# shubhamchandak94/Spring

Measured on AMD Instinct MI355X. Metric: Mreads/s through reorder stage, higher is better.
Workload: dtype u64; 1 GPU; 100000000 x 150 bp single-end synthetic reads per GPU (uniform genome 600000000 bp, 25x coverage, 1.0% substitutions, 50% reverse-complemented), inputs resident in HBM as .dna records; reads_per_gpu=100000000, read_len=150, chains=65536, num_thr=8, parallelism=single GPU, unmatched=13958636, singletons=12720853, rounds=1984, chain_groups=2

## Files before the change

include/spring_reorder.h:

```cpp
#ifndef SPRING_REORDER_H_
#define SPRING_REORDER_H_

#include <stddef.h>
#include <stdint.h>

#ifdef __cplusplus
extern "C" {
#endif

#define SPRING_REORDER_E_ARG (-1)
#define SPRING_REORDER_E_IO (-2)
#define SPRING_REORDER_E_HIP (-3)
#define SPRING_REORDER_E_STATE (-4)

typedef struct spring_reorder_ctx spring_reorder_ctx;

typedef struct {
  int32_t device;
  uint32_t num_chains;
  int32_t num_thr;
  int32_t collect_stats;
  int32_t time_search;
  int32_t force_literal_update;
  int32_t rounds_per_sync;
  int32_t long_budget;
  int32_t first_shifts;
  int32_t seed_wide;
  int32_t tab_scale;
  int32_t search_wpb;
  int32_t dbg_search_lds;
  int32_t dbg_apply_lds;
  int32_t fused;
  int32_t deep_bins;
  int32_t num_devices;
  int32_t devices[8];
  int32_t mg_host_transport;
  int32_t table_mode;
  int32_t plan0[6];
  int32_t plan1[6];
  int32_t long_min;
  int32_t long_blocks;
  int32_t debug;
  int32_t long_split;
  int32_t entry_flags;
  int32_t out_writers;
  int32_t alternatives;
  int32_t phases;
  int32_t known_absent;
} spring_reorder_opts;

typedef struct {
  uint64_t n_reads, n_matched, n_single, unmatched;
  uint64_t probes, keyok, cands, hits, iterations, rounds, lost;
  uint64_t numkeys[2], dict_numreads[2];
  double ms_unpack, ms_dict, ms_chains, ms_finalize, ms_total;
  double ms_search_kernel;
  uint64_t search_launches;
  uint64_t device_bytes;
  double ms_exchange, ms_resolve_mark;
  uint64_t chains;
  uint64_t deep_pool;
  uint64_t long_searches;
  uint64_t table_minz;
  uint64_t table_marked_lines;
  uint64_t long_splits;
  uint64_t alternatives;
  uint64_t phases;
  double ms_search_busy;
} spring_reorder_stats;

void spring_reorder_default_opts(spring_reorder_opts *o);
const char *spring_reorder_last_error(void);
void spring_reorder_trim_pool(void);

int spring_reorder_run(const char *temp_dir, uint32_t max_readlen, int32_t num_thr, int32_t paired_end,
                       uint32_t num_reads_clean_0, uint32_t num_reads_clean_1,
                       const spring_reorder_opts *opts );

int spring_reorder_create(spring_reorder_ctx **ctx, const spring_reorder_opts *opts);
void spring_reorder_destroy(spring_reorder_ctx *ctx);

int spring_reorder_load_dna(spring_reorder_ctx *ctx, const uint8_t *dna, size_t nbytes, uint32_t n,
                            uint32_t max_readlen);

int spring_reorder_load_dna_device(spring_reorder_ctx *ctx, const void *d_dna, size_t nbytes, uint32_t n,
                                   uint32_t max_readlen, int32_t fixed_len);

int spring_reorder_build_dict(spring_reorder_ctx *ctx);

int spring_reorder_run_chains(spring_reorder_ctx *ctx);
int spring_reorder_auto_chains(spring_reorder_ctx *ctx, uint32_t *chains, int32_t *deep);

typedef struct {
  uint32_t num_reads[2], num_reads_clean[2], num_reads_N[2];
  uint32_t max_readlen;
  uint32_t pad;
  double ms_device;
} spring_fastq_info;
int spring_reorder_load_fastq(spring_reorder_ctx *ctx, const uint8_t *fastq_1, size_t nbytes_1, const uint8_t *fastq_2,
                              size_t nbytes_2 , spring_fastq_info *info);
int spring_reorder_fastq_N(spring_reorder_ctx *ctx, int32_t which, uint8_t *n_dna, size_t cap, size_t *nbytes,
                           uint32_t *order_N, uint32_t *count);

int spring_reorder_mg_begin(spring_reorder_ctx *ctx, uint32_t rank, uint32_t world, uint32_t total_chains, void *d_prop);
int spring_reorder_mg_search(spring_reorder_ctx *ctx);
int spring_reorder_mg_slice(spring_reorder_ctx *ctx, void **d_prop, size_t *slice_off, size_t *slice_bytes,
                            size_t *total_bytes);
int spring_reorder_mg_slices(spring_reorder_ctx *ctx, void **d_prop, size_t slice_off[2], size_t slice_bytes[2],
                             size_t *total_bytes, uint32_t *count);
int spring_reorder_mg_apply(spring_reorder_ctx *ctx, int32_t check_alive, uint32_t *alive);
int spring_reorder_mg_end(spring_reorder_ctx *ctx);
int spring_reorder_debug_check_seed_state(spring_reorder_ctx *ctx, int32_t group, uint64_t *violations);
int spring_reorder_mg_exchange_virtual(spring_reorder_ctx **ctxs, uint32_t world);

#define SPRING_RCCL_ID_BYTES 128
typedef struct spring_mg_comm spring_mg_comm;
typedef int (*spring_mg_allgather_fn)(void *host_buf, size_t slice_off, size_t slice_bytes, size_t total_bytes,
                                      void *user);
int spring_mg_rccl_unique_id(void *id128);
int spring_mg_comm_create_rccl(spring_mg_comm **comm, int32_t device, const void *id128, uint32_t rank, uint32_t world);
int spring_mg_comm_create_host(spring_mg_comm **comm, spring_mg_allgather_fn fn, void *user, uint32_t rank,
                               uint32_t world);
void spring_mg_comm_destroy(spring_mg_comm *comm);
int spring_reorder_mg_run(spring_reorder_ctx *ctx, spring_mg_comm *comm, uint32_t total_chains);

int spring_reorder_finalize(spring_reorder_ctx *ctx);

int spring_reorder_get_stats(spring_reorder_ctx *ctx, spring_reorder_stats *st);

int spring_reorder_download(spring_reorder_ctx *ctx, uint32_t *order, char *rc, char *flag, int64_t *pos,
                            uint16_t *rlen, uint32_t *order_s, uint64_t *tid_off, uint64_t *tid_off_s);
int spring_reorder_tid_split(spring_reorder_ctx *ctx, uint64_t *mid, uint64_t *mid_s);

int spring_reorder_emit_dna(spring_reorder_ctx *ctx, int32_t tid, uint8_t *dst, size_t cap, size_t *nbytes);

int spring_reorder_dict_lookup(spring_reorder_ctx *ctx, int32_t which, const uint64_t *keys, uint32_t nkeys,
                               uint32_t *bin_size, uint32_t *bin_ids, size_t ids_cap);

int spring_reorder_download_reads(spring_reorder_ctx *ctx, uint64_t *limbs , uint16_t *len);

int spring_order_invert_se(const uint32_t *order, uint32_t n, uint32_t *order_array, double *kernel_ms);
int spring_order_invert_pe(const uint32_t *order, uint32_t n, uint32_t *order_array, double *kernel_ms);
int spring_order_correct(uint32_t *order, uint64_t m, const uint32_t *order_N, uint32_t nN, uint32_t n_clean,
                         double *kernel_ms);
int spring_order_pe_encode(const uint32_t *order, uint32_t n, uint32_t *new_order, double *kernel_ms);

int spring_fastq_reorder(const uint8_t *fastq, size_t nbytes, const uint32_t *order, uint32_t n, uint8_t *out,
                         size_t out_cap, size_t *out_bytes, double *kernel_ms);

#define SPRING_SYNTH_REPEATS 0x80000000u
#define SPRING_SYNTH_PAIRED 0x40000000u
#define SPRING_SYNTH_GENOMIC 0x20000000u
size_t spring_synth_dna_bytes(uint32_t n, uint32_t L);
int spring_synth_dna_host(uint8_t *dst, uint32_t n, uint32_t L, uint64_t G, uint64_t seed, uint32_t err_ppm);
int spring_synth_genome_host(uint8_t *dst, uint64_t G, uint64_t seed, uint32_t flags);
int spring_synth_dna_device(void *d_dst, uint32_t n, uint32_t L, uint64_t G, uint64_t seed, uint32_t err_ppm);
int spring_reorder_load_synth(spring_reorder_ctx *ctx, uint32_t n, uint32_t L, uint64_t G, uint64_t seed,
                              uint32_t err_ppm);
int spring_reorder_download_dna(spring_reorder_ctx *ctx, uint8_t *dst, size_t cap);

#ifdef __cplusplus
}
#endif
#endif
```

spring_amd/_lib.py:

```python
import ctypes as C
import os

HERE = os.path.dirname(os.path.abspath(__file__))
LIB_PATH = os.environ.get("SPRING_AMD_LIB") or os.path.join(HERE, "lib", "libspring_reorder_hip.so")

EXPORTS = [
    "spring_reorder_default_opts", "spring_reorder_last_error", "spring_reorder_trim_pool", "spring_reorder_run", "spring_reorder_create",
    "spring_reorder_destroy", "spring_reorder_load_dna", "spring_reorder_load_dna_device",
    "spring_reorder_build_dict", "spring_reorder_run_chains", "spring_reorder_auto_chains", "spring_reorder_finalize",
    "spring_reorder_mg_begin", "spring_reorder_mg_search", "spring_reorder_mg_slice", "spring_reorder_mg_slices",
    "spring_reorder_mg_apply",
    "spring_reorder_mg_end", "spring_reorder_mg_exchange_virtual", "spring_reorder_debug_check_seed_state",
    "spring_mg_rccl_unique_id", "spring_mg_comm_create_rccl", "spring_mg_comm_create_host", "spring_mg_comm_destroy",
    "spring_reorder_mg_run",
    "spring_reorder_get_stats", "spring_reorder_download", "spring_reorder_tid_split", "spring_reorder_emit_dna",
    "spring_reorder_dict_lookup", "spring_reorder_download_reads", "spring_synth_dna_bytes",
    "spring_reorder_load_fastq", "spring_reorder_fastq_N",
    "spring_order_invert_se", "spring_order_invert_pe", "spring_order_correct", "spring_order_pe_encode",
    "spring_fastq_reorder",
    "spring_synth_dna_host", "spring_synth_genome_host", "spring_synth_dna_device", "spring_reorder_load_synth", "spring_reorder_download_dna",
    "spring_encoder_create", "spring_encoder_destroy", "spring_encoder_set_split_tables", "spring_encoder_encode_reorder", "spring_encoder_download",
    "spring_encoder_download_seq_packed", "spring_encoder_get_info", "spring_reorder_encode_run", "spring_encoder_encode_host", "spring_encoder_run",
]

STREAMS_EXPORTS = [
    "spring_streams_create", "spring_streams_destroy", "spring_streams_from_encoder", "spring_streams_from_host",
    "spring_streams_download", "spring_streams_get_info", "spring_streams_run",
]
STREAMS_NUM = 9

DECODE_EXPORTS = [
    "spring_decode_create", "spring_decode_destroy", "spring_decode_seq_from_encoder", "spring_decode_seq_from_host",
    "spring_decode_seq_from_files", "spring_decode_from_streams", "spring_decode_from_host", "spring_decode_from_files",
    "spring_decode_download", "spring_decode_get_info",
]


class Opts(C.Structure):
    _fields_ = [("device", C.c_int32), ("num_chains", C.c_uint32), ("num_thr", C.c_int32),
                ("collect_stats", C.c_int32), ("time_search", C.c_int32), ("force_literal_update", C.c_int32),
                ("rounds_per_sync", C.c_int32), ("long_budget", C.c_int32),
                ("first_shifts", C.c_int32), ("seed_wide", C.c_int32), ("tab_scale", C.c_int32),
                ("search_wpb", C.c_int32), ("dbg_search_lds", C.c_int32), ("dbg_apply_lds", C.c_int32),
                ("fused", C.c_int32), ("deep_bins", C.c_int32),
                ("num_devices", C.c_int32), ("devices", C.c_int32 * 8), ("mg_host_transport", C.c_int32),
                ("table_mode", C.c_int32), ("plan0", C.c_int32 * 6), ("plan1", C.c_int32 * 6), ("long_min", C.c_int32),
                ("long_blocks", C.c_int32), ("debug", C.c_int32), ("long_split", C.c_int32), ("entry_flags", C.c_int32),
                ("out_writers", C.c_int32), ("alternatives", C.c_int32), ("phases", C.c_int32), ("known_absent", C.c_int32)]


class FastqInfo(C.Structure):
    _fields_ = [("num_reads", C.c_uint32 * 2), ("num_reads_clean", C.c_uint32 * 2), ("num_reads_N", C.c_uint32 * 2),
                ("max_readlen", C.c_uint32), ("pad", C.c_uint32), ("ms_device", C.c_double)]


class EncoderInfo(C.Structure):
    _fields_ = ([(k, C.c_uint64) for k in ("n_aligned", "n_total", "seq_len", "noise_bytes", "n_noisepos",
                                           "unaligned_bytes", "len_unaligned", "num_contigs")]
                + [(k, C.c_uint32) for k in ("matched_s", "matched_N", "align_passes", "max_bin")]
                + [("ms_device", C.c_double), ("ms_phase", C.c_double * 8)])

    def asdict(self):
        d = {}
        for k, _ in self._fields_:
            v = getattr(self, k)
            d[k] = list(v) if hasattr(v, "__len__") else v
        return d


class StreamsInfo(C.Structure):
    _fields_ = ([("num_units", C.c_uint64), ("num_blocks", C.c_uint64), ("bytes", C.c_uint64 * STREAMS_NUM),
                 ("flag_count", C.c_uint64 * 5), ("pos_escapes", C.c_uint64), ("n_aligned", C.c_uint64),
                 ("ms_device", C.c_double), ("ms_file", C.c_double)])

    def asdict(self):
        d = {}
        for k, _ in self._fields_:
            v = getattr(self, k)
            d[k] = list(v) if hasattr(v, "__len__") else v
        return d


class DecodeInfo(C.Structure):
    _fields_ = ([(k, C.c_uint64) for k in ("seq_len", "first_block", "num_blocks", "num_units")]
                + [("bases", C.c_uint64 * 2)]
                + [(k, C.c_uint64) for k in ("n_aligned", "n_unaligned", "pos_escapes")]
                + [("ms_device", C.c_double), ("ms_file", C.c_double)])

    def asdict(self):
        d = {}
        for k, _ in self._fields_:
            v = getattr(self, k)
            d[k] = list(v) if hasattr(v, "__len__") else v
        return d


class Stats(C.Structure):
    _fields_ = ([(k, C.c_uint64) for k in ("n_reads", "n_matched", "n_single", "unmatched", "probes", "keyok",
                                          "cands", "hits", "iterations", "rounds", "lost")]
                + [("numkeys", C.c_uint64 * 2), ("dict_numreads", C.c_uint64 * 2)]
                + [(k, C.c_double) for k in ("ms_unpack", "ms_dict", "ms_chains", "ms_finalize", "ms_total",
                                             "ms_search_kernel")]
                + [("search_launches", C.c_uint64), ("device_bytes", C.c_uint64),
                   ("ms_exchange", C.c_double), ("ms_resolve_mark", C.c_double), ("chains", C.c_uint64),
                   ("deep_pool", C.c_uint64), ("long_searches", C.c_uint64),
                   ("table_minz", C.c_uint64), ("table_marked_lines", C.c_uint64), ("long_splits", C.c_uint64), ("alternatives", C.c_uint64), ("phases", C.c_uint64),
                   ("ms_search_busy", C.c_double)])

    def asdict(self):
        d = {}
        for k, _ in self._fields_:
            v = getattr(self, k)
            d[k] = list(v) if hasattr(v, "__len__") else v
        return d


MG_ALLGATHER_FN = C.CFUNCTYPE(C.c_int, C.c_void_p, C.c_size_t, C.c_size_t, C.c_size_t, C.c_void_p)

_lib = None


def lib():
    global _lib
    if _lib is not None:
        return _lib
    if not os.path.exists(LIB_PATH):
        raise RuntimeError(
            "spring_amd: %s is missing. Build it with `python -m spring_amd.build` "
            "(or __graft_entry__.build()); there is no CPU fallback." % LIB_PATH)
    L = C.CDLL(LIB_PATH)
    vp, u8p = C.c_void_p, C.c_void_p
    L.spring_reorder_default_opts.argtypes = [C.POINTER(Opts)]
    L.spring_reorder_last_error.restype = C.c_char_p
    L.spring_reorder_trim_pool.restype = None
    L.spring_reorder_run.argtypes = [C.c_char_p, C.c_uint32, C.c_int32, C.c_int32, C.c_uint32, C.c_uint32,
                                     C.POINTER(Opts)]
    L.spring_reorder_create.argtypes = [C.POINTER(vp), C.POINTER(Opts)]
    L.spring_reorder_destroy.argtypes = [vp]
    L.spring_reorder_destroy.restype = None
    L.spring_reorder_load_dna.argtypes = [vp, u8p, C.c_size_t, C.c_uint32, C.c_uint32]
    L.spring_reorder_load_dna_device.argtypes = [vp, vp, C.c_size_t, C.c_uint32, C.c_uint32, C.c_int32]
    L.spring_reorder_build_dict.argtypes = [vp]
    L.spring_reorder_run_chains.argtypes = [vp]
    L.spring_reorder_auto_chains.argtypes = [vp, C.POINTER(C.c_uint32), C.POINTER(C.c_int32)]
    L.spring_reorder_finalize.argtypes = [vp]
    L.spring_reorder_mg_begin.argtypes = [vp, C.c_uint32, C.c_uint32, C.c_uint32, vp]
    L.spring_reorder_mg_search.argtypes = [vp]
    L.spring_reorder_mg_slice.argtypes = [vp, C.POINTER(vp), C.POINTER(C.c_size_t), C.POINTER(C.c_size_t), C.POINTER(C.c_size_t)]
    L.spring_reorder_mg_slices.argtypes = [vp, C.POINTER(vp), C.POINTER(C.c_size_t), C.POINTER(C.c_size_t), C.POINTER(C.c_size_t),
                                           C.POINTER(C.c_uint32)]
    L.spring_reorder_debug_check_seed_state.argtypes = [vp, C.c_int32, C.POINTER(C.c_uint64)]
    L.spring_reorder_mg_apply.argtypes = [vp, C.c_int32, C.POINTER(C.c_uint32)]
    L.spring_reorder_mg_end.argtypes = [vp]
    L.spring_reorder_mg_exchange_virtual.argtypes = [C.POINTER(vp), C.c_uint32]
    L.spring_mg_rccl_unique_id.argtypes = [vp]
    L.spring_mg_comm_create_rccl.argtypes = [C.POINTER(vp), C.c_int32, vp, C.c_uint32, C.c_uint32]
    L.spring_mg_comm_create_host.argtypes = [C.POINTER(vp), MG_ALLGATHER_FN, vp, C.c_uint32, C.c_uint32]
    L.spring_mg_comm_destroy.argtypes = [vp]
    L.spring_mg_comm_destroy.restype = None
    L.spring_reorder_mg_run.argtypes = [vp, vp, C.c_uint32]
    L.spring_reorder_get_stats.argtypes = [vp, C.POINTER(Stats)]
    L.spring_reorder_download.argtypes = [vp] + [vp] * 8
    L.spring_reorder_tid_split.argtypes = [vp, vp, vp]
    L.spring_reorder_emit_dna.argtypes = [vp, C.c_int32, u8p, C.c_size_t, C.POINTER(C.c_size_t)]
    L.spring_reorder_dict_lookup.argtypes = [vp, C.c_int32, vp, C.c_uint32, vp, vp, C.c_size_t]
    L.spring_reorder_download_reads.argtypes = [vp, vp, vp]
    L.spring_reorder_load_fastq.argtypes = [vp, vp, C.c_size_t, vp, C.c_size_t, C.POINTER(FastqInfo)]
    L.spring_reorder_fastq_N.argtypes = [vp, C.c_int32, vp, C.c_size_t, C.POINTER(C.c_size_t), vp, C.POINTER(C.c_uint32)]
    L.spring_order_invert_se.argtypes = [vp, C.c_uint32, vp, C.POINTER(C.c_double)]
    L.spring_order_invert_pe.argtypes = [vp, C.c_uint32, vp, C.POINTER(C.c_double)]
    L.spring_fastq_reorder.argtypes = [u8p, C.c_size_t, vp, C.c_uint32, u8p, C.c_size_t, C.POINTER(C.c_size_t),
                                       C.POINTER(C.c_double)]
    L.spring_order_pe_encode.argtypes = [vp, C.c_uint32, vp, C.POINTER(C.c_double)]
    L.spring_order_correct.argtypes = [vp, C.c_uint64, vp, C.c_uint32, C.c_uint32, C.POINTER(C.c_double)]
    L.spring_synth_dna_bytes.restype = C.c_size_t
    L.spring_synth_dna_bytes.argtypes = [C.c_uint32, C.c_uint32]
    L.spring_synth_dna_host.argtypes = [u8p, C.c_uint32, C.c_uint32, C.c_uint64, C.c_uint64, C.c_uint32]
    L.spring_synth_genome_host.argtypes = [u8p, C.c_uint64, C.c_uint64, C.c_uint32]
    L.spring_synth_dna_device.argtypes = [vp, C.c_uint32, C.c_uint32, C.c_uint64, C.c_uint64, C.c_uint32]
    L.spring_reorder_load_synth.argtypes = [vp, C.c_uint32, C.c_uint32, C.c_uint64, C.c_uint64, C.c_uint32]
    L.spring_reorder_download_dna.argtypes = [vp, u8p, C.c_size_t]
    L.spring_encoder_create.argtypes = [C.c_int32, C.POINTER(vp)]
    L.spring_encoder_destroy.argtypes = [vp]
    L.spring_encoder_destroy.restype = None
    L.spring_encoder_encode_reorder.argtypes = [vp, vp, u8p, C.c_uint64, vp, C.c_uint32, C.POINTER(EncoderInfo)]
    L.spring_encoder_download.argtypes = [vp] + [vp] * 9
    L.spring_encoder_download_seq_packed.argtypes = [vp, vp, vp]
    L.spring_encoder_encode_host.argtypes = [vp, C.c_uint32, C.c_int32, vp, u8p, C.c_uint64, vp, vp, vp, vp, vp, u8p,
                                             C.c_uint64, vp, C.c_uint32, u8p, C.c_uint64, vp, C.c_uint32,
                                             C.POINTER(EncoderInfo)]
    L.spring_encoder_run.argtypes = [C.c_char_p, C.c_uint32, C.c_int32, C.c_uint32, C.c_uint32, C.c_int32,
                                     C.POINTER(EncoderInfo)]
    L.spring_encoder_get_info.argtypes = [vp, C.POINTER(EncoderInfo)]
    L.spring_reorder_encode_run.argtypes = [C.c_char_p, C.c_uint32, C.c_int32, C.c_int32, C.c_uint32, C.c_uint32,
                                            C.c_uint32, C.POINTER(Opts), C.POINTER(EncoderInfo)]
    L.spring_streams_create.argtypes = [C.c_int32, C.POINTER(vp)]
    L.spring_streams_destroy.argtypes = [vp]
    L.spring_streams_destroy.restype = None
    L.spring_streams_from_encoder.argtypes = [vp, vp, C.c_uint32, C.c_int32, C.c_int32, C.c_uint32, C.c_int32,
                                              C.POINTER(StreamsInfo)]
    L.spring_streams_from_host.argtypes = [vp, vp, vp, C.c_uint64, vp, C.c_uint64, vp, C.c_uint64, vp, vp, C.c_uint64, vp,
                                           C.c_uint64, C.c_uint32, C.c_int32, C.c_int32, C.c_uint32, C.POINTER(StreamsInfo)]
    L.spring_streams_download.argtypes = [vp, C.c_int32, vp, vp]
    L.spring_streams_get_info.argtypes = [vp, C.POINTER(StreamsInfo)]
    L.spring_streams_run.argtypes = [C.c_char_p, C.c_uint32, C.c_int32, C.c_int32, C.c_uint32, C.c_int32,
                                     C.POINTER(StreamsInfo)]
    L.spring_decode_create.argtypes = [C.c_int32, C.POINTER(vp)]
    L.spring_decode_destroy.argtypes = [vp]
    L.spring_decode_destroy.restype = None
    L.spring_decode_seq_from_encoder.argtypes = [vp, vp]
    L.spring_decode_seq_from_host.argtypes = [vp, C.c_int32, vp, vp, vp]
    L.spring_decode_seq_from_files.argtypes = [vp, C.c_char_p, C.c_int32]
    L.spring_decode_from_streams.argtypes = [vp, vp, C.POINTER(DecodeInfo)]
    L.spring_decode_from_host.argtypes = [vp, vp, vp, C.c_uint32, C.c_uint32, C.c_uint32, C.c_int32, C.c_int32,
                                          C.c_uint32, C.POINTER(DecodeInfo)]
    L.spring_decode_from_files.argtypes = [vp, C.c_char_p, C.c_uint32, C.c_uint32, C.c_uint32, C.c_int32, C.c_int32,
                                           C.c_uint32, C.POINTER(DecodeInfo)]
    L.spring_decode_download.argtypes = [vp, C.c_int32, vp, vp]
    L.spring_decode_get_info.argtypes = [vp, C.POINTER(DecodeInfo)]
    for name in DECODE_EXPORTS:
        if name != "spring_decode_destroy":
            getattr(L, name).restype = C.c_int
    for name in STREAMS_EXPORTS:
        if name != "spring_streams_destroy":
            getattr(L, name).restype = C.c_int
    for name in EXPORTS:
        if name not in ("spring_reorder_last_error", "spring_reorder_destroy", "spring_synth_dna_bytes",
                        "spring_reorder_default_opts", "spring_reorder_trim_pool", "spring_encoder_destroy",
                        "spring_mg_comm_destroy"):
            getattr(L, name).restype = C.c_int
    _lib = L
    return L
```

spring_amd/csrc/reorder_device.h:

```cpp
#ifndef SPRING_REORDER_DEVICE_H_
#define SPRING_REORDER_DEVICE_H_

#include <hip/hip_runtime.h>
#include <stdint.h>

namespace sr {

constexpr int MAX_READ_LEN = 511;
constexpr int MAX_SEARCH = 1000;
constexpr int THRESH = 4;
constexpr uint32_t DEEP_BIN = 16;
constexpr uint32_t MID_BIN = 64;
constexpr uint32_t BIG_BIN = 256;
constexpr uint32_t CHUNK = 64;
constexpr uint32_t MARK_BLOCK = 256;
constexpr uint32_t MC_WAVES_PER_BLOCK = MARK_BLOCK / 4 + 3;
constexpr int UBLK_SHIFT = 12;
constexpr int LDS_PAD = 10;
constexpr int LDS_LIMBS = 16 + 2 * LDS_PAD;

enum { MODE_SEARCH = 0, MODE_NEED_SEED = 1 };
enum { PROP_NONE = 0, PROP_MATCH = 1, PROP_SEED = 2, PROP_FRESH = 3  };
enum { PK_NONE = 0, PK_MATCH = 1, PK_SEED = 2, PK_NOSEED = 4, PK_DONE = 5 };
constexpr unsigned long long PK_CURSOR_BIT = 1ull << 35;
constexpr unsigned long long PK_WILLNEED_BIT = 1ull << 36;
constexpr int PK_ALT_SHIFT = 37;
constexpr uint32_t ALT_MAX_READS = (1u << 27) - 1;
constexpr uint32_t ALT_KEY = 1u << 28;

struct __attribute__((aligned(16))) ChainHot {
  long long ref_pos;
  int32_t ref_len;
  uint32_t e_slot;
  uint32_t prev, first_rid;
  uint32_t n_emit, n_single;
  uint32_t s_slot;
  uint32_t num_reads_thr, num_unmatched_past;
  uint32_t prop_rid;
  union {
    struct {
      uint32_t done : 1, prev_unmatched : 1, left_search : 1, stop_searching : 1;
      uint32_t mode : 1, retrying : 1, finishing : 1, cursor_writer : 1;
      uint32_t cnt_buf : 1;
      uint32_t cnt_wide : 1;
      uint32_t prop_kind : 2;
      uint32_t prop_rev : 3;
      uint32_t prop_shift : 9;
    };
    uint32_t flags;
  };
  uint32_t alt1;
  uint32_t pad[2];
};
static_assert(sizeof(ChainHot) == 64, "ChainHot must be one 64-byte line");

struct __attribute__((aligned(64))) Chain {
  ChainHot h;
  uint64_t ref[16];
  uint64_t revref[16];
  uint64_t st_probes, st_keyok, st_cands, st_iter, st_lost, st_hits, n_unmatched, st_long ;
#ifdef SR_PHASE_TIMING
  uint64_t pt[64];
#endif
};
#ifndef SR_PHASE_TIMING
static_assert(sizeof(Chain) == 384, "Chain layout");
#endif

struct Globals {
  long long cursor;
  uint32_t alive;
  uint32_t e_alloc;
  uint32_t s_alloc;
  uint32_t pad;
  long long cursor_b;
};

struct TabView {
  const uint4 *buck;
  int bshift;
  int minz;
  int lshift;
};
constexpr uint32_t TAG_MARK = 0xfffffffcu;
constexpr int MINZ_HEAVY = 12;
constexpr int MINZ_K = 16;
constexpr int MINZ_WL = 32;

constexpr int LONG_MAX_BINS = 1024;
constexpr int LONG_MAX_PARTS = 64;
struct LongHead {
  uint32_t nb, nparts, best_single, bestrid;
  uint32_t bestpart, pad[3];
  uint32_t blo[LONG_MAX_PARTS + 4];
  uint32_t rescode[LONG_MAX_PARTS], resrid[LONG_MAX_PARTS];
  uint32_t capped[LONG_MAX_PARTS];
};
struct DevParams {
  const uint64_t *reads;
  const uint16_t *lens;
  uint32_t n;
  int L, W, S, Lpad, maxshift, uniform_len;
  int plan[2][6];
  int seed_wide;
  int deep_bins;
  int search_wpb;
  int dbg_search_lds, dbg_apply_lds;
  int wl;
  int dstart[2], dend[2];
  uint32_t numkeys[2];
  TabView tab;
  const ulonglong2 *urec[2];
  const uint32_t *ids[2];
  uint32_t *epos[2];
  uint32_t idmask;
  const ulonglong2 *sig[2];
  uint64_t *taken;
  uint32_t *ublk;
  uint32_t *resv;
  uint32_t *needy;
  uint32_t *needy_cnt;
  uint32_t *needy_cnt_next;
  int fused;
  int alts;
  int mc;
  int ka, ka_lo;
  uint32_t *ord;
  uint4 *ord_cnt;
  uint32_t *longq;
  int long_budget, long_min, long_blocks, long_part;
  uint32_t *lctl, *lparts;
  struct LongHead *lhead;
  uint2 *lbin;
  uint16_t *lbcode;
  uint32_t lbin_stride;
#ifdef SR_PHASE_TIMING
  unsigned long long *dbg;
#endif
  Globals *glob;
  long long *cursor;
  uint32_t K, c0, Ktot;
  int phases;
  uint32_t g0, Kg, g0_other, Kg_other;
  uint32_t gg0, gKg, gKg_other;
  uint32_t seed_lo, seed_hi;
  uint32_t nb_lo, nb_hi;
  const uint64_t *taken_other;
  uint32_t *won, *won_other;
  unsigned long long *prop;
  uint32_t *alive_wave;
  Chain *chains;
  int4 *cnt;
  uint32_t *cnt8;
  uint4 *e_rec; uint2 *e_chunk;
  uint32_t *s_rec; uint2 *s_chunk;
  uint32_t *f_order; char *f_rc; char *f_flag; long long *f_pos; uint16_t *f_len; uint32_t *f_order_s;
};

void launch_unpack(hipStream_t st, const uint8_t *dna, const uint64_t *off, uint32_t n, int L, int W, int S,
                   uint32_t rec_fixed, uint64_t *reads, uint16_t *lens, uint32_t *bad_len = nullptr);
void launch_flag_in_dict(hipStream_t st, const uint16_t *lens, uint32_t n, int dend, uint32_t *flag);
void launch_keys(hipStream_t st, const uint64_t *reads, const uint16_t *lens, const uint32_t *slot, uint32_t n,
                 int S, int dstart, int dend, uint64_t *keys, uint32_t *vals);
struct DictBuild {
  const uint32_t *ustart, *ucount, *ids;
  ulonglong2 *urec;
  uint32_t *deep, *ndeep;
};
void launch_tab_insert(hipStream_t st, const uint64_t *mhash, const uint64_t *mval, uint64_t nmerged, DictBuild d0,
                       DictBuild d1, uint32_t *fpt, int bshift);
void launch_minz_prepare(hipStream_t st, const uint64_t *mhash, const uint64_t *mval, uint64_t nmerged, DictBuild d0,
                         DictBuild d1, int lshift, uint32_t *bucket, uint64_t *tagpay);
void launch_tab_insert_minz(hipStream_t st, const uint32_t *bucket_sorted, const uint64_t *tagpay_sorted, uint64_t nmerged,
                            uint32_t *fpt, int bshift, uint32_t *marked);
hipError_t sort_pairs_u32_u64(hipStream_t st, void *tmp, size_t &tmp_bytes, const uint32_t *kin, uint32_t *kout,
                              const uint64_t *vin, uint64_t *vout, size_t n, unsigned end_bit);
hipError_t merge_by_hash(hipStream_t st, void *tmp, size_t &tmp_bytes, const uint64_t *k0, const uint64_t *k1,
                         const uint64_t *v0, const uint64_t *v1, uint64_t *kout, uint64_t *vout, size_t n0, size_t n1);
void launch_iota_tag(hipStream_t st, uint64_t *v, uint64_t n, uint64_t tag);
void launch_build_epos(hipStream_t st, const uint32_t *ids, uint64_t m, uint32_t *epos);
void launch_trim_bins(hipStream_t st, const uint32_t *deep, const uint32_t *ndeep, uint32_t ndeep_host,
                      ulonglong2 *urec, const uint32_t *ids, const uint64_t *taken, ulonglong2 *sig ,
                      uint32_t *epos = nullptr );
void launch_build_sig(hipStream_t st, const uint32_t *ids, uint64_t m, const uint64_t *reads, int S, int W, ulonglong2 *sig);
void launch_dict_lookup(hipStream_t st, TabView tab, const ulonglong2 *urec, int which,
                        const uint64_t *reads, int S, int dstart, int dend, const uint64_t *keys, uint32_t nkeys,
                        uint32_t *start, uint32_t *count);
void launch_fill_u32(hipStream_t st, uint32_t *p, uint64_t n, uint32_t v);
void launch_init_taken(hipStream_t st, uint64_t *taken, uint64_t nwords, uint32_t n, uint32_t *ublk);
void launch_init_chains(hipStream_t st, const DevParams &P, bool seeds = true);
void launch_check_seed_state(hipStream_t st, const DevParams &P, uint64_t nwords, uint64_t hi, unsigned long long *bad);
void launch_search(hipStream_t st, const DevParams &P, bool stats);
void launch_apply(hipStream_t st, const DevParams &P, bool literal);
void launch_round(hipStream_t st, const DevParams &P, bool stats, bool mg);
void launch_mg_resolve(hipStream_t st, const DevParams &P);
void launch_mg_mark(hipStream_t st, const DevParams &P);
void launch_ph_mark(hipStream_t st, const DevParams &P);
void launch_delay(hipStream_t st, uint32_t microseconds);
void launch_chain_summary(hipStream_t st, const DevParams &P, uint2 *sum, unsigned long long *tot );
void launch_scatter(hipStream_t st, const DevParams &P, uint64_t cap_m, uint64_t cap_s, const uint64_t *off_m,
                    const uint64_t *off_s);
void launch_rec_size(hipStream_t st, const uint32_t *order, const uint16_t *lens, uint64_t cnt, uint32_t *sz);
void launch_emit_dna(hipStream_t st, const uint64_t *reads, const uint16_t *lens, int S, const uint32_t *order,
                     const char *rc, uint64_t cnt, const uint64_t *off, uint32_t rec_fixed, uint8_t *dst);
void launch_synth(hipStream_t st, uint8_t *dst, uint32_t n, uint32_t L, uint64_t G, uint64_t seed, uint32_t thr24);

constexpr int NL_CHUNK_BYTES = 4096;
void launch_nl_count(hipStream_t st, const uint8_t *t, uint64_t nbytes, uint32_t *blk_cnt, uint64_t nblk);
void launch_nl_fill(hipStream_t st, const uint8_t *t, uint64_t nbytes, const uint64_t *blk_off, uint64_t *line_end,
                    uint64_t nblk);
void launch_read_info(hipStream_t st, const uint8_t *t, const uint64_t *line_end, uint64_t nreads, uint32_t *len,
                      uint32_t *fclean, uint32_t *szc, uint32_t *fN, uint32_t *szN, uint32_t *lenc, uint32_t *err);
void launch_pack_reads(hipStream_t st, const uint8_t *t, const uint64_t *line_end, uint64_t nreads, const uint32_t *len,
                       const uint32_t *fclean, const uint32_t *cidx, const uint64_t *coff, const uint32_t *nidx,
                       const uint64_t *noff, uint32_t cidx_base, uint64_t coff_base, uint32_t file_read_base,
                       uint8_t *out_clean, uint64_t *out_off, uint8_t *out_N, uint32_t *out_orderN, uint64_t *out_offN);
hipError_t reduce_max_u32(hipStream_t st, void *tmp, size_t &tmp_bytes, const uint32_t *in, uint32_t *out, size_t n);
hipError_t reduce_min_u32(hipStream_t st, void *tmp, size_t &tmp_bytes, const uint32_t *in, uint32_t *out, size_t n);

hipError_t sort_pairs(hipStream_t st, void *tmp, size_t &tmp_bytes, const uint64_t *kin, uint64_t *kout,
                      const uint32_t *vin, uint32_t *vout, size_t n, unsigned end_bit);
hipError_t rle(hipStream_t st, void *tmp, size_t &tmp_bytes, const uint64_t *in, size_t n, uint64_t *uniq,
               uint32_t *counts, uint32_t *nruns);
hipError_t excl_scan_u32(hipStream_t st, void *tmp, size_t &tmp_bytes, const uint32_t *in, uint32_t *out, size_t n);
hipError_t excl_scan_u32_to_u64(hipStream_t st, void *tmp, size_t &tmp_bytes, const uint32_t *in, uint64_t *out,
                                size_t n);

}
#endif
```

spring_amd/csrc/reorder_kernels.hip:

```cpp
#include <cstdlib>
#include <cstring>
#include <hip/hip_runtime.h>
#include <rocprim/rocprim.hpp>

#include "reorder_device.h"
#include "synth_common.h"

namespace sr {


__device__ __forceinline__ uint64_t mix64(uint64_t x) {
  x ^= x >> 33; x *= 0xff51afd7ed558ccdull; x ^= x >> 33; x *= 0xc4ceb9fe1a85ec53ull; x ^= x >> 33;
  return x;
}

__device__ __forceinline__ void wave_sync() {
  __builtin_amdgcn_fence(__ATOMIC_SEQ_CST, "wavefront");
  __builtin_amdgcn_wave_barrier();
}

__device__ __forceinline__ int uni_i32(int v) { return __builtin_amdgcn_readfirstlane(v); }
template <class T>
__device__ __forceinline__ T *uni_ptr(T *p) {
  const uint64_t a = reinterpret_cast<uint64_t>(p);
// ... 31 lines not shown
__device__ __forceinline__ uint64_t lds_window(const uint64_t *s, int bitpos) {
  int li = bitpos >> 6, off = bitpos & 63;
  uint64_t lo = s[li], hi = s[li + 1];
  return off ? (lo >> off) | (hi << (64 - off)) : lo;
}

__device__ __forceinline__ bool is_taken(const uint64_t *__restrict__ taken, uint32_t rid) {
  return (taken[rid >> 6] >> (rid & 63)) & 1ull;
}
__device__ __forceinline__ bool entry_dead(const DevParams &P, uint32_t &r, bool &trimmable) {
  if (P.idmask != 0xffffffffu) {
    const bool f = (r >> 31) != 0;
    r &= 0x7fffffffu;
    trimmable = f;
    if (f || P.phases != 2) return f;
    return is_taken(P.taken, r);
  }
  const bool d = is_taken(P.taken, r);
  trimmable = d && (P.phases != 2 || is_taken(P.taken_other, r));
  return d;
}

__device__ __forceinline__ uint32_t fp30_of(uint64_t h) {
  const uint32_t f = (uint32_t)h & 0x3fffffffu;
  return f == 0u ? 1u : f == 0x3fffffffu ? 0x3ffffffeu : f;
}
__device__ __forceinline__ uint64_t bucket_of(uint64_t h, int bshift) { return h >> bshift; }
__device__ __forceinline__ uint64_t bucket_mask(int bshift) { return (1ull << (64 - bshift)) - 1; }
__device__ __forceinline__ uint64_t unmix64(uint64_t x) {
  x ^= x >> 33; x *= 0x9cb4b2f8129337dbull; x ^= x >> 33; x *= 0x4f74430c22a54005ull; x ^= x >> 33;
  return x;
}
__device__ __forceinline__ uint32_t fmix32(uint32_t x) {
  x ^= x >> 16; x *= 0x85ebca6bu; x ^= x >> 13; x *= 0xc2b2ae35u; x ^= x >> 16;
  return x;
}
__device__ __forceinline__ uint32_t kmer_order(uint32_t x) {
  uint32_t r = __builtin_bitreverse32(x);
  r = ~(((r >> 1) & 0x55555555u) | ((r & 0x55555555u) << 1));
  return ((x < r ? x : r) ^ 0x5bd1e995u) * 0x9e3779b1u;
}
__device__ __forceinline__ uint32_t minz_of_key(uint64_t key) {
  uint32_t m = 0xffffffffu;
#pragma unroll
  for (int q = 0; q <= MINZ_WL - MINZ_K; q++) m = min(m, kmer_order((uint32_t)(key >> (2 * q))));
  return fmix32(m);
}
__device__ __forceinline__ uint64_t tab_home(const TabView &T, uint64_t h, uint32_t mz) {
  return T.minz ? (((uint64_t)(mz >> T.lshift) << 2) | ((h >> 30) & 3ull)) : bucket_of(h, T.bshift);
}
__device__ __forceinline__ uint64_t tab_redirect_x(uint32_t x32, int bshift) { return mix64(0x6a09e667f3bcc908ull ^ x32) >> bshift; }
__device__ __forceinline__ uint64_t tab_redirect(const TabView &T, uint64_t h) {
  return tab_redirect_x(fp30_of(h) | ((uint32_t)((h >> 30) & 3ull) << 30), T.bshift);
}
template <bool MZ = false>
__device__ __forceinline__ int tab_find(const TabView &T, uint64_t h, uint32_t mz, int l, int skip,
                                        uint32_t &pay, bool &other) {
  const uint32_t mine = (fp30_of(h) << 2) | ((uint32_t)l << 1), theirs = mine ^ 2u;
  const uint64_t bmask = bucket_mask(T.bshift);
  uint64_t b = MZ ? tab_home(T, h, mz) : bucket_of(h, T.bshift);
  bool first = MZ && T.minz != 0;
  for (;;) {
#if defined(SR_TAGS_NT)
    typedef uint32_t u32x4_t __attribute__((ext_vector_type(4)));
    const u32x4_t tv = __builtin_nontemporal_load(reinterpret_cast<const u32x4_t *>(&T.buck[b * 2]));
    const uint4 t = make_uint4(tv.x, tv.y, tv.z, tv.w);
#elif defined(SR_TAGS_SC)
    typedef uint32_t u32x4_t __attribute__((ext_vector_type(4)));
    u32x4_t tv;
    asm volatile("global_load_dwordx4 %0, %1, off sc0 sc1\n\ts_waitcnt vmcnt(0)" : "=v"(tv) : "v"(&T.buck[b * 2]) : "memory");
    const uint4 t = make_uint4(tv.x, tv.y, tv.z, tv.w);
#else
    const uint4 t = T.buck[b * 2];
#endif
    if (MZ && first) {
      first = false;
      if (t.x == TAG_MARK) { b = tab_redirect(T, h); continue; }
    }
    other = other || (t.x & ~1u) == theirs || (t.y & ~1u) == theirs || (t.z & ~1u) == theirs || t.w != 0;
    uint32_t m = (uint32_t)((t.x & ~1u) == mine) | ((uint32_t)((t.y & ~1u) == mine) << 1) |
                 ((uint32_t)((t.z & ~1u) == mine) << 2) | ((uint32_t)((t.w & ~1u) == mine) << 3);
    const int c = __popc(m);
    if (c > skip) {
      for (; skip > 0; skip--) m &= m - 1;
      const int I = __ffs((int)m) - 1;
      const uint32_t Tg = I == 0 ? t.x : I == 1 ? t.y : I == 2 ? t.z : t.w;
      pay = reinterpret_cast<const uint32_t *>(T.buck)[b * 8 + 4 + I];
      return 1 + (int)(Tg & 1u);
    }
    if (t.w == 0) return 0;
    skip -= c;
    b = (b + 1) & bmask;
  }
}
__device__ __forceinline__ uint64_t read_window(const uint64_t *__restrict__ r, int S, int dstart, int klen2) {
  const int bitpos = 2 * dstart, li = bitpos >> 6, off = bitpos & 63;
  uint64_t v = r[li] >> off;
  if (off && li + 1 < S) v |= r[li + 1] << (64 - off);
  if (klen2 < 64) v &= (1ull << klen2) - 1;
  return v;
}

#ifdef SR_PHASE_TIMING
#ifndef SR_PT_LONG
#define SR_PT_LONG 1000000
#endif
__shared__ uint32_t g_pt_lds[66];
#define PT(k)                                                                                         \
  do {                                                                                                \
    const uint32_t t_ = (uint32_t)clock64();                                                          \
    const unsigned long long ex_ = __ballot(1);                                                       \
    if ((int)(threadIdx.x & 63) == __ffsll(ex_) - 1) {                                                \
      g_pt_lds[(k)] += t_ - g_pt_lds[64]; g_pt_lds[32 + (k)] += 1u; g_pt_lds[64] = t_;                 \
    }                                                                                                 \
  } while (0)
#define PTW(k) do { asm volatile("s_waitcnt vmcnt(0) lgkmcnt(0)" ::: "memory"); PT(k); } while (0)
#define PT_FLUSH(c)                                                              \
  do {                                                                           \
    wave_sync();                                                                 \
    (c)->pt[threadIdx.x & 63] += g_pt_lds[threadIdx.x & 63];                     \
  } while (0)
#else
#define PT(k) do {} while (0)
#define PTW(k) do {} while (0)
#define PT_FLUSH(c) do {} while (0)
#endif

__global__ void k_unpack(const uint8_t *__restrict__ dna, const uint64_t *__restrict__ off, uint32_t n,
                         int L, int W, int S, uint32_t rec_fixed, uint64_t *__restrict__ reads,
                         uint16_t *__restrict__ lens, uint32_t *__restrict__ bad_len) {
  uint64_t t = (uint64_t)blockIdx.x * blockDim.x + threadIdx.x;
  uint64_t i = t / (uint32_t)S;
  int j = (int)(t % (uint32_t)S);
  if (i >= n) return;
  uint64_t o = off ? off[i] : i * (uint64_t)rec_fixed;
  uint32_t len = (uint32_t)dna[o] | ((uint32_t)dna[o + 1] << 8);
  if (bad_len && !off && len != (uint32_t)L) {
    if (j == 0) *bad_len = 1u;
    len = (uint32_t)L;
  }
  if (j == 0) lens[i] = (uint16_t)len;
  uint32_t nb = (len + 3) / 4;
  uint64_t v = 0;
  if (j < W) {
#pragma unroll
    for (int b = 0; b < 8; b++) {
      uint32_t pos = 8u * j + b;
      if (pos < nb) v |= (uint64_t)dna[o + 2 + pos] << (8 * b);
    }
  }
  reads[i * S + j] = v;
}

__global__ void k_flag_in_dict(const uint16_t *__restrict__ lens, uint32_t n, int dend,
                               uint32_t *__restrict__ flag) {
  uint32_t i = blockIdx.x * blockDim.x + threadIdx.x;
  if (i < n) flag[i] = lens[i] > dend ? 1u : 0u;
}

__global__ void k_keys(const uint64_t *__restrict__ reads, const uint16_t *__restrict__ lens,
                       const uint32_t *__restrict__ slot , uint32_t n,
                       int S, int dstart, int dend, uint64_t *__restrict__ keys, uint32_t *__restrict__ vals) {
  uint32_t i = blockIdx.x * blockDim.x + threadIdx.x;
  if (i >= n) return;
  if (slot && !(lens[i] > dend)) return;
  const uint64_t *r = reads + (uint64_t)i * S;
  int bitpos = 2 * dstart, nbits = 2 * (dend - dstart + 1);
  int li = bitpos >> 6, offb = bitpos & 63;
  uint64_t v = r[li] >> offb;
  if (offb && li + 1 < S) v |= r[li + 1] << (64 - offb);
  if (nbits < 64) v &= (1ull << nbits) - 1;
  uint32_t o = slot ? slot[i] : i;
  keys[o] = mix64(v);
  vals[o] = i;
}

template <bool OVERFLOW>
__global__ void k_tab_insert(const uint64_t *__restrict__ mhash, const uint64_t *__restrict__ mval, uint64_t nm,
                             DictBuild d0, DictBuild d1, uint32_t *fpt, int bshift) {
  const uint64_t i = (uint64_t)blockIdx.x * blockDim.x + threadIdx.x;
  if (i >= nm) return;
  const uint64_t h = mhash[i];
  const uint64_t b0 = bucket_of(h, bshift);
  int rank = 0;
  while (rank < 4 && i > (uint64_t)rank && bucket_of(mhash[i - 1 - rank], bshift) == b0) rank++;
  if (OVERFLOW != (rank >= 4)) return;
  const uint64_t mv = mval[i];
  const uint32_t l = (uint32_t)(mv >> 63), u = (uint32_t)mv;
  const DictBuild &d = l ? d1 : d0;
  const uint32_t st = d.ustart[u], cn = d.ucount[u];
  const bool single = cn == 1;
  const uint32_t tag = (fp30_of(h) << 2) | (l << 1) | (single ? 1u : 0u);
  const uint32_t pay = single ? d.ids[st] : u;
  if (cn >= DEEP_BIN) d.deep[atomicAdd(d.ndeep, 1u)] = u;
  if (cn >= BIG_BIN) atomicAdd(d.ndeep + 1, cn);
  if (cn >= MID_BIN) atomicAdd(d.ndeep + 2, cn);
  d.urec[u] = make_ulonglong2(unmix64(h), (uint64_t)st | ((uint64_t)cn << 32));
  if (!OVERFLOW) {
    fpt[b0 * 8 + rank] = tag;
    fpt[b0 * 8 + 4 + rank] = pay;
    return;
  }
  const uint64_t bmask = bucket_mask(bshift);
  uint64_t b = (b0 + 1) & bmask;
  for (;;) {
    uint32_t *bk = fpt + b * 8;
    for (int sl = 0; sl < 4; sl++) {
      if (atomicCAS(bk + sl, 0u, tag) == 0u) {
        bk[4 + sl] = pay;
        return;
      }
    }
    b = (b + 1) & bmask;
  }
}

__global__ void k_minz_prepare(const uint64_t *__restrict__ mhash, const uint64_t *__restrict__ mval, uint64_t nm,
                               DictBuild d0, DictBuild d1, int lshift, uint32_t *__restrict__ bucket,
                               uint64_t *__restrict__ tagpay) {
  const uint64_t i = (uint64_t)blockIdx.x * blockDim.x + threadIdx.x;
  if (i >= nm) return;
  const uint64_t h = mhash[i], key = unmix64(h);
  const uint64_t mv = mval[i];
  const uint32_t l = (uint32_t)(mv >> 63), u = (uint32_t)mv;
  const DictBuild &d = l ? d1 : d0;
  const uint32_t st = d.ustart[u], cn = d.ucount[u];
  const bool single = cn == 1;
  const uint32_t tag = (fp30_of(h) << 2) | (l << 1) | (single ? 1u : 0u);
  const uint32_t pay = single ? d.ids[st] : u;
  if (cn >= DEEP_BIN) d.deep[atomicAdd(d.ndeep, 1u)] = u;
  if (cn >= BIG_BIN) atomicAdd(d.ndeep + 1, cn);
  if (cn >= MID_BIN) atomicAdd(d.ndeep + 2, cn);
  d.urec[u] = make_ulonglong2(key, (uint64_t)st | ((uint64_t)cn << 32));
  bucket[i] = ((minz_of_key(key) >> lshift) << 2) | (uint32_t)((h >> 30) & 3ull);
  tagpay[i] = (uint64_t)tag | ((uint64_t)pay << 32);
}
template <bool SECOND>
__global__ void k_tab_insert_minz(const uint32_t *__restrict__ bk, const uint64_t *__restrict__ tp, uint64_t nm,
                                  uint32_t *fpt, int bshift, uint32_t *marked ) {
  const uint64_t i = (uint64_t)blockIdx.x * blockDim.x + threadIdx.x;
  if (i >= nm) return;
  const uint32_t b0 = bk[i], line = b0 >> 2;
  int back = 0;
  while (back <= MINZ_HEAVY && i > (uint64_t)back && (bk[i - 1 - back] >> 2) == line) back++;
  bool heavy = back > MINZ_HEAVY;
  if (!heavy) {
    const uint64_t at = i - back + MINZ_HEAVY;
    heavy = at < nm && (bk[at] >> 2) == line;
  }
  int rank = 0;
  if (!heavy) while (rank < 4 && rank < back && bk[i - 1 - rank] == b0) rank++;
  const uint64_t w = tp[i];
  const uint32_t tag = (uint32_t)w, pay = (uint32_t)(w >> 32);
  if (!SECOND) {
    if (heavy) {
      if (back == 0) {
        for (int s = 0; s < 4; s++) fpt[((uint64_t)line * 4 + s) * 8] = TAG_MARK;
        atomicAdd(marked, 1u);
      }
    } else if (rank < 4) {
      fpt[(uint64_t)b0 * 8 + rank] = tag;
      fpt[(uint64_t)b0 * 8 + 4 + rank] = pay;
    }
    return;
  }
  if (!heavy && rank < 4) return;
  const uint64_t bmask = bucket_mask(bshift);
  uint64_t b = heavy ? tab_redirect_x((tag >> 2) | ((b0 & 3u) << 30), bshift) : (((uint64_t)b0 + 1) & bmask);
  for (;;) {
    uint32_t *bk = fpt + b * 8;
    for (int sl = 0; sl < 4; sl++) {
      if (atomicCAS(bk + sl, 0u, tag) == 0u) {
        bk[4 + sl] = pay;
        return;
      }
    }
    b = (b + 1) & bmask;
  }
}
__global__ void k_iota_tag(uint64_t *v, uint64_t n, uint64_t tag) {
  const uint64_t i = (uint64_t)blockIdx.x * blockDim.x + threadIdx.x;
  if (i < n) v[i] = i | tag;
}

__global__ __launch_bounds__(256) void k_trim_bins(const uint32_t *__restrict__ deep, const uint32_t *__restrict__ ndeep,
                                                   ulonglong2 *__restrict__ urec, uint32_t *__restrict__ ids,
                                                   const uint64_t *__restrict__ taken, ulonglong2 *__restrict__ sig ,
                                                   uint32_t *__restrict__ epos ) {
  const uint32_t i = blockIdx.x * 4 + (threadIdx.x >> 6);
  const int lane = threadIdx.x & 63;
  if (i >= *ndeep) return;
  const uint32_t u = deep[i];
  const ulonglong2 rec = urec[u];
  const uint32_t start = (uint32_t)rec.y, count = (uint32_t)(rec.y >> 32);
  uint32_t w = 0;
  for (uint32_t base = 0; base < count; base += 64) {
    const uint32_t j = base + lane;
    const uint32_t r = j < count ? ids[start + j] : 0u;
    const bool live = j < count && (epos ? !(r >> 31) : !is_taken(taken, r));
    ulonglong2 sg = make_ulonglong2(0, 0);
    if (sig && live) sg = sig[start + j];
    const uint64_t m = __ballot(live);
    const uint32_t pos = w + (uint32_t)__popcll(m & ((1ull << lane) - 1));
    if (live && pos != j) {
      ids[start + pos] = r;
      if (sig) sig[start + pos] = sg;
      if (epos) epos[r] = start + pos;
    }
    w += (uint32_t)__popcll(m);
  }
  if (lane == 0 && w != count) urec[u].y = (uint64_t)start | ((uint64_t)w << 32);
}

__global__ void k_dict_lookup(TabView tab, const ulonglong2 *__restrict__ urec, int which,
                              const uint64_t *__restrict__ reads, int S, int dstart, int klen2,
                              const uint64_t *__restrict__ keys, uint32_t nkeys, uint32_t *__restrict__ start,
                              uint32_t *__restrict__ count) {
  uint32_t i = blockIdx.x * blockDim.x + threadIdx.x;
  if (i >= nkeys) return;
  const uint64_t key = keys[i], h = mix64(key);
  const uint32_t mz = tab.minz ? minz_of_key(key) : 0u;
  uint32_t s = 0, c = 0xffffffffu;
  for (int skip = 0;; skip++) {
    uint32_t pay;
    bool other = false;
    const int kind = tab_find<true>(tab, h, mz, which, skip, pay, other);
    if (kind == 0) break;
    if (kind == 1) {
      const ulonglong2 r = urec[pay];
      if (r.x != key) continue;
      s = (uint32_t)r.y; c = (uint32_t)(r.y >> 32);
      break;
    }
    if (read_window(reads + (uint64_t)pay * S, S, dstart, klen2) != key) continue;
    s = pay; c = 1u | 0x80000000u;
    break;
  }
  start[i] = s;
  count[i] = c;
// ... 2077 lines not shown
  const uint64_t m = __ballot(local);
  uint32_t wbase = 0;
  if ((threadIdx.x & 63) == 0 && m) wbase = atomicAdd(&s_n, (uint32_t)__popcll(m));
  wbase = (uint32_t)__shfl((int)wbase, 0, 64);
  if (local) P.ord[(size_t)blk * MARK_BLOCK + wbase + (uint32_t)__popcll(m & ((1ull << (threadIdx.x & 63)) - 1))] = cid - P.c0;
  __syncthreads();
  if (threadIdx.x == 0) P.ord_cnt[blk] = make_uint4(0u, 0u, s_n, 0u);
}

__global__ void k_chain_summary(DevParams P, uint2 *__restrict__ sum, unsigned long long *__restrict__ tot ) {
  const uint32_t i = blockIdx.x * blockDim.x + threadIdx.x;
  uint64_t v[8] = {0, 0, 0, 0, 0, 0, 0, 0};
  if (i < P.K) {
    const Chain &c = P.chains[i];
    sum[i] = make_uint2(c.h.n_emit, c.h.n_single);
    v[0] = c.n_unmatched; v[1] = c.st_probes; v[2] = c.st_keyok; v[3] = c.st_cands; v[4] = c.st_iter; v[5] = c.st_lost; v[6] = c.st_hits; v[7] = c.st_long;
  }
#pragma unroll
  for (int k = 0; k < 8; k++) {
    const uint64_t w = wave_sum_u64(v[k]);
    if ((threadIdx.x & 63) == 0 && w) atomicAdd(&tot[k], (unsigned long long)w);
  }
}

__global__ void k_scatter_matched(DevParams P, uint64_t cap, const uint64_t *__restrict__ off_m) {
  uint64_t i = (uint64_t)blockIdx.x * blockDim.x + threadIdx.x;
  if (i >= cap) return;
  const uint2 ci = P.e_chunk[i / CHUNK];
  if (ci.x == 0xffffffffu) return;
  const uint32_t seq = ci.y + (uint32_t)(i % CHUNK);
  if (seq >= P.chains[ci.x].h.n_emit) return;
  const uint4 r = P.e_rec[i];
  const uint64_t d = off_m[ci.x] + seq;
  P.f_order[d] = r.x; P.f_rc[d] = (char)(r.y & 0xffu); P.f_flag[d] = (char)((r.y >> 8) & 0xffu);
  P.f_pos[d] = (long long)((unsigned long long)r.z | ((unsigned long long)r.w << 32));
  P.f_len[d] = P.uniform_len ? (uint16_t)P.L : P.lens[r.x];
}
__global__ void k_scatter_single(DevParams P, uint64_t cap, const uint64_t *__restrict__ off_s) {
  uint64_t i = (uint64_t)blockIdx.x * blockDim.x + threadIdx.x;
  if (i >= cap) return;
  const uint2 ci = P.s_chunk[i / CHUNK];
  if (ci.x == 0xffffffffu) return;
  const uint32_t seq = ci.y + (uint32_t)(i % CHUNK);
  if (seq >= P.chains[ci.x].h.n_single) return;
  P.f_order_s[off_s[ci.x] + seq] = P.s_rec[i];
}

__global__ void k_rec_size(const uint32_t *__restrict__ order, const uint16_t *__restrict__ lens, uint64_t cnt,
                           uint32_t *__restrict__ sz) {
  uint64_t i = (uint64_t)blockIdx.x * blockDim.x + threadIdx.x;
  if (i < cnt) sz[i] = 2u + ((uint32_t)lens[order[i]] + 3u) / 4u;
}
__global__ void k_emit_dna(const uint64_t *__restrict__ reads, const uint16_t *__restrict__ lens, int S,
                           const uint32_t *__restrict__ order, const char *__restrict__ rc, uint64_t cnt,
                           const uint64_t *__restrict__ off, uint32_t rec_fixed, uint8_t *__restrict__ dst) {
  uint64_t i = (uint64_t)blockIdx.x * blockDim.x + threadIdx.x;
  if (i >= cnt) return;
  const uint32_t rid = order[i];
  const uint32_t len = lens[rid];
  const uint64_t *r = reads + (uint64_t)rid * S;
  uint8_t *o = dst + (off ? off[i] : i * (uint64_t)rec_fixed);
  o[0] = (uint8_t)(len & 0xff); o[1] = (uint8_t)(len >> 8);
  const uint32_t nb = (len + 3) / 4;
  const bool rev = rc && rc[i] == 'r';
  for (uint32_t b = 0; b < nb; b++) {
    uint32_t v = 0;
    if (!rev) v = (uint32_t)(r[b >> 3] >> (8 * (b & 7))) & 0xffu;
    else {
      for (uint32_t q = 0; q < 4; q++) {
        uint32_t j = 4 * b + q;
        if (j < len) {
          uint32_t s = len - 1 - j;
          uint32_t code = (uint32_t)(r[s >> 5] >> (2 * (s & 31))) & 3u;
          v |= (3u - code) << (2 * q);
        }
      }
    }
    o[2 + b] = (uint8_t)v;
  }
}

__device__ __forceinline__ uint32_t emit_dna_byte(const uint64_t *__restrict__ r, uint32_t len, bool rev, uint32_t o) {
  if (o == 0) return len & 0xffu;
  if (o == 1) return len >> 8;
  const uint32_t b = o - 2;
  if (!rev) return (uint32_t)(r[b >> 3] >> (8 * (b & 7))) & 0xffu;
  const int lo = (int)len - 4 - 4 * (int)b;
  uint32_t w8;
  if (lo >= 0) {
    const int p = 2 * lo, li = p >> 6, sh = p & 63;
    uint64_t v = r[li] >> sh;
    if (sh > 56) v |= r[li + 1] << (64 - sh);
    w8 = (uint32_t)v & 0xffu;
  } else {
    w8 = ((uint32_t)r[0] << (-2 * lo)) & 0xffu;
  }
  const uint32_t x = ~w8 & 0xffu;
  uint32_t v = ((x & 3u) << 6) | ((x & 0xcu) << 2) | ((x >> 2) & 0xcu) | (x >> 6);
  if (lo < 0) v &= 0xffu >> (-2 * lo);
  return v;
}
__global__ void k_emit_dna_fixed(const uint64_t *__restrict__ reads, const uint16_t *__restrict__ lens, int S,
                                 const uint32_t *__restrict__ order, const char *__restrict__ rc, uint64_t cnt,
                                 uint32_t rec, uint8_t *__restrict__ dst) {
  const uint64_t W = (uint64_t)blockIdx.x * blockDim.x + threadIdx.x, total = cnt * rec;
  if (4 * W >= total) return;
  uint64_t i = 4 * W / rec;
  uint32_t o = (uint32_t)(4 * W - i * rec);
  uint32_t word = 0;
  const uint32_t nbytes = (uint32_t)(total - 4 * W < 4 ? total - 4 * W : 4);
  uint64_t ci = ~0ull;
  const uint64_t *r = nullptr;
  uint32_t len = 0;
  bool rev = false;
  for (uint32_t k = 0; k < nbytes; k++) {
    if (i != ci) {
      const uint32_t rid = order[i];
      len = lens[rid];
      r = reads + (uint64_t)rid * S;
      rev = rc && rc[i] == 'r';
      ci = i;
    }
    word |= emit_dna_byte(r, len, rev, o) << (8 * k);
    if (++o == rec) { o = 0; i++; }
  }
  if (nbytes == 4) *reinterpret_cast<uint32_t *>(dst + 4 * W) = word;
  else for (uint32_t k = 0; k < nbytes; k++) dst[4 * W + k] = (uint8_t)(word >> (8 * k));
}

__global__ void k_synth(uint8_t *__restrict__ dst, uint32_t n, uint32_t L, uint64_t G, uint64_t seed,
                        uint32_t thr24) {
  uint64_t i = (uint64_t)blockIdx.x * blockDim.x + threadIdx.x;
  if (i >= n) return;
  const uint32_t rec = 2u + (L + 3) / 4;
  uint8_t *o = dst + i * rec;
  uint64_t pos; uint32_t rc;
  syn_read_params(seed, G, L, i, (thr24 & SYN_PAIRED_FLAG) ? n / 2 : 0, &pos, &rc);
  o[0] = (uint8_t)(L & 0xff); o[1] = (uint8_t)(L >> 8);
  for (uint32_t b = 0; b < (L + 3) / 4; b++) {
    uint32_t v = 0;
    for (uint32_t q = 0; q < 4; q++) {
      uint32_t j = 4 * b + q;
      if (j < L) v |= syn_nat_to_spring(syn_read_base(seed, G, L, thr24, i, j, pos, rc)) << (2 * q);
    }
    o[2 + b] = (uint8_t)v;
  }
}

#define GRID1(n, bs) dim3((unsigned)(((uint64_t)(n) + (bs) - 1) / (bs)))

void launch_unpack(hipStream_t st, const uint8_t *dna, const uint64_t *off, uint32_t n, int L, int W, int S,
                   uint32_t rec_fixed, uint64_t *reads, uint16_t *lens, uint32_t *bad_len) {
  if (!n) return;
  uint64_t tot = (uint64_t)n * S;
  hipLaunchKernelGGL(k_unpack, GRID1(tot, 256), dim3(256), 0, st, dna, off, n, L, W, S, rec_fixed, reads, lens, bad_len);
}
void launch_flag_in_dict(hipStream_t st, const uint16_t *lens, uint32_t n, int dend, uint32_t *flag) {
  hipLaunchKernelGGL(k_flag_in_dict, GRID1(n, 256), dim3(256), 0, st, lens, n, dend, flag);
}
void launch_keys(hipStream_t st, const uint64_t *reads, const uint16_t *lens, const uint32_t *slot, uint32_t n,
                 int S, int dstart, int dend, uint64_t *keys, uint32_t *vals) {
  hipLaunchKernelGGL(k_keys, GRID1(n, 256), dim3(256), 0, st, reads, lens, slot, n, S, dstart, dend, keys, vals);
}
void launch_tab_insert(hipStream_t st, const uint64_t *mhash, const uint64_t *mval, uint64_t nmerged, DictBuild d0,
                       DictBuild d1, uint32_t *fpt, int bshift) {
  if (!nmerged) return;
  hipLaunchKernelGGL(k_tab_insert<false>, GRID1(nmerged, 256), dim3(256), 0, st, mhash, mval, nmerged, d0, d1, fpt, bshift);
  hipLaunchKernelGGL(k_tab_insert<true>, GRID1(nmerged, 256), dim3(256), 0, st, mhash, mval, nmerged, d0, d1, fpt, bshift);
}
void launch_minz_prepare(hipStream_t st, const uint64_t *mhash, const uint64_t *mval, uint64_t nmerged, DictBuild d0,
                         DictBuild d1, int lshift, uint32_t *bucket, uint64_t *tagpay) {
  if (!nmerged) return;
  hipLaunchKernelGGL(k_minz_prepare, GRID1(nmerged, 256), dim3(256), 0, st, mhash, mval, nmerged, d0, d1, lshift, bucket, tagpay);
}
void launch_tab_insert_minz(hipStream_t st, const uint32_t *bucket_sorted, const uint64_t *tagpay_sorted, uint64_t nmerged,
                            uint32_t *fpt, int bshift, uint32_t *marked) {
  if (!nmerged) return;
  hipLaunchKernelGGL(k_tab_insert_minz<false>, GRID1(nmerged, 256), dim3(256), 0, st, bucket_sorted, tagpay_sorted, nmerged, fpt, bshift, marked);
  hipLaunchKernelGGL(k_tab_insert_minz<true>, GRID1(nmerged, 256), dim3(256), 0, st, bucket_sorted, tagpay_sorted, nmerged, fpt, bshift, marked);
}
void launch_iota_tag(hipStream_t st, uint64_t *v, uint64_t n, uint64_t tag) {
  if (!n) return;
  hipLaunchKernelGGL(k_iota_tag, GRID1(n, 256), dim3(256), 0, st, v, n, tag);
}
void launch_trim_bins(hipStream_t st, const uint32_t *deep, const uint32_t *ndeep, uint32_t ndeep_host,
                      ulonglong2 *urec, const uint32_t *ids, const uint64_t *taken, ulonglong2 *sig, uint32_t *epos) {
  if (!ndeep_host) return;
  hipLaunchKernelGGL(k_trim_bins, GRID1(ndeep_host, 4), dim3(256), 0, st, deep, ndeep, urec, const_cast<uint32_t *>(ids), taken, sig, epos);
}
void launch_dict_lookup(hipStream_t st, TabView tab, const ulonglong2 *urec, int which,
                        const uint64_t *reads, int S, int dstart, int dend, const uint64_t *keys, uint32_t nkeys,
                        uint32_t *start, uint32_t *count) {
  if (!nkeys) return;
  hipLaunchKernelGGL(k_dict_lookup, GRID1(nkeys, 256), dim3(256), 0, st, tab, urec, which, reads, S, dstart,
                     2 * (dend - dstart + 1), keys, nkeys, start, count);
}
void launch_fill_u32(hipStream_t st, uint32_t *p, uint64_t n, uint32_t v) {
  if (!n) return;
  hipLaunchKernelGGL(k_fill_u32, GRID1(n, 256), dim3(256), 0, st, p, n, v);
}
__global__ void k_check_seed_state(DevParams P, uint64_t nwords, uint64_t hi, unsigned long long *bad) {
  const uint64_t w = (uint64_t)blockIdx.x * blockDim.x + threadIdx.x;
  if (w >= nwords) return;
  const long long top = *P.cursor;
  const uint64_t v = P.taken[w];
  const long long first = (long long)w * 64;
  const long long a = max(max(top + 1, (long long)P.seed_lo), first), e = min((long long)hi, first + 64);
  if (a < e) {
    const int nb = (int)(e - a);
    const uint64_t must = (nb >= 64 ? ~0ull : ((1ull << nb) - 1ull)) << (int)(a - first);
    if ((v & must) != must) atomicAdd(&bad[0], 1ull);
  }
  constexpr int WPB_ = 1 << (UBLK_SHIFT - 6);
  const long long blk = (long long)(w / WPB_);
  if ((w % WPB_) == 0 && top >= (long long)P.seed_lo && blk >= (long long)(P.seed_lo >> UBLK_SHIFT) && blk < (top >> UBLK_SHIFT)) {
    int cnt = 0;
    for (int k = 0; k < WPB_; k++) cnt += __popcll(~P.taken[w + k]);
    if ((uint32_t)cnt != P.ublk[blk]) atomicAdd(&bad[1], 1ull);
  }
}
void launch_check_seed_state(hipStream_t st, const DevParams &P, uint64_t nwords, uint64_t hi, unsigned long long *bad) {
  if (!nwords) return;
  hipLaunchKernelGGL(k_check_seed_state, GRID1(nwords, 256), dim3(256), 0, st, P, nwords, hi, bad);
}
void launch_init_taken(hipStream_t st, uint64_t *taken, uint64_t nwords, uint32_t n, uint32_t *ublk) {
  if (!nwords) return;
  hipLaunchKernelGGL(k_init_taken, GRID1(nwords, 256), dim3(256), 0, st, taken, nwords, n, ublk);
}
#define NP_DISPATCH(CALL)                                  \
  do {                                                     \
    const int np_ = P.Lpad / 64;                           \
    if (np_ <= 1) { CALL(1); } else if (np_ == 2) { CALL(2); } else if (np_ == 3) { CALL(3); } \
    else if (np_ == 4) { CALL(4); } else { CALL(8); }      \
  } while (0)

void launch_init_chains(hipStream_t st, const DevParams &P, bool seeds) {
  if (seeds && P.Ktot) hipLaunchKernelGGL(k_init_seeds, GRID1(P.Ktot, 256), dim3(256), 0, st, P);
  if (!P.Kg) return;
  if (P.ord) hipLaunchKernelGGL(k_init_ord, GRID1(P.gKg, MARK_BLOCK), dim3(MARK_BLOCK), 0, st, P);
#define CALL(N) hipLaunchKernelGGL(k_init_chains<N>, dim3((P.Kg + 3) / 4), dim3(256), 0, st, P)
  NP_DISPATCH(CALL);
#undef CALL
}
template <int WPB>
static void launch_search_wpb(hipStream_t st, const DevParams &P, bool stats) {
  const dim3 g((P.K + WPB - 1) / WPB), b(64 * WPB);
  const size_t dyn = (size_t)P.dbg_search_lds;
  if (stats) hipLaunchKernelGGL((k_search<true, WPB>), g, b, dyn, st, P);
  else hipLaunchKernelGGL((k_search<false, WPB>), g, b, dyn, st, P);
}
void launch_search(hipStream_t st, const DevParams &P, bool stats) {
  if (!P.K) return;
#ifdef SR_DEV_PROD_ONLY
  (void)st; (void)stats; abort();
#else
  if (P.search_wpb == 1) launch_search_wpb<1>(st, P, stats);
  else if (P.search_wpb == 2) launch_search_wpb<2>(st, P, stats);
  else launch_search_wpb<4>(st, P, stats);
#endif
}
void launch_apply(hipStream_t st, const DevParams &P, bool literal) {
  if (!P.K) return;
#ifdef SR_DEV_PROD_ONLY
  (void)st; (void)literal; abort();
#else
  const dim3 g((P.K + 3) / 4), b(256);
  if (literal) { hipLaunchKernelGGL((k_apply<8, true>), g, b, 0, st, P); return; }
#define CALL(N) hipLaunchKernelGGL((k_apply<N, false>), g, b, (size_t)P.dbg_apply_lds, st, P)
  NP_DISPATCH(CALL);
#undef CALL
#endif
}
void launch_round(hipStream_t st, const DevParams &P, bool stats, bool mg) {
  if (!P.K || !P.Kg) return;
  const dim3 g(P.Kg), b(64);
  const size_t dyn = (size_t)P.dbg_search_lds;
  if (P.mc && !stats && !P.deep_bins) {
    const uint32_t nseg = (P.c0 + P.g0 + P.Kg + MARK_BLOCK - 1) / MARK_BLOCK - (P.c0 + P.g0) / MARK_BLOCK;
    const dim3 g4(nseg * MC_WAVES_PER_BLOCK);
    if (P.Lpad <= 192) {
      if (P.ka) {
        if (mg) hipLaunchKernelGGL((k_round_mc<3, true, true>), g4, b, 0, st, P);
        else hipLaunchKernelGGL((k_round_mc<3, false, true>), g4, b, 0, st, P);
      } else if (mg) hipLaunchKernelGGL((k_round_mc<3, true, false>), g4, b, 0, st, P);
      else hipLaunchKernelGGL((k_round_mc<3, false, false>), g4, b, 0, st, P);
    } else {
      if (mg) hipLaunchKernelGGL((k_round_mc_long<true>), g4, b, 0, st, P);
      else hipLaunchKernelGGL((k_round_mc_long<false>), g4, b, 0, st, P);
    }
    return;
  }
#ifdef SR_DEV_PROD_ONLY
  if (stats || mg || P.deep_bins || P.Lpad > 192) abort();
  hipLaunchKernelGGL((k_round<3, false, false, false>), g, b, dyn, st, P);
#else
#define RCALL2(N, KERN)                                                                      \
  do {                                                                                       \
    if (mg) { if (stats) hipLaunchKernelGGL((KERN<N, true, true>), g, b, dyn, st, P);        \
              else hipLaunchKernelGGL((KERN<N, false, true>), g, b, dyn, st, P); }           \
    else { if (stats) hipLaunchKernelGGL((KERN<N, true, false>), g, b, dyn, st, P);          \
           else hipLaunchKernelGGL((KERN<N, false, false>), g, b, dyn, st, P); }             \
  } while (0)
#define RCALL(N) do { if (P.deep_bins) RCALL2(N, k_round_t); else RCALL2(N, k_round_nt); } while (0)
  if (P.deep_bins && !stats && P.long_budget > 0 && P.longq) {
#define LCALL(N) do { if (mg) hipLaunchKernelGGL((k_round_tl<N, true>), g, b, dyn, st, P); \
                      else hipLaunchKernelGGL((k_round_tl<N, false>), g, b, dyn, st, P); } while (0)
    if (P.Lpad <= 192) LCALL(3); else LCALL(8);
#undef LCALL
    const uint32_t lb = (uint32_t)P.long_blocks;
    if (4 * P.maxshift <= 512) hipLaunchKernelGGL(k_long_list<8>, dim3(std::min<uint32_t>(P.K, 3 * lb)), dim3(512), 0, st, P);
    else hipLaunchKernelGGL(k_long_list<LONG_WAVES>, dim3(std::min<uint32_t>(P.K, lb)), dim3(64 * LONG_WAVES), 0, st, P);
    hipLaunchKernelGGL(k_long_scan, dim3(std::min<uint32_t>(P.K * 4, 5 * lb)), dim3(64 * SCAN_WAVES), 0, st, P);
    hipLaunchKernelGGL(k_long_fin, dim3(std::min<uint32_t>((P.K + 3) / 4, lb)), dim3(256), 0, st, P, 1);
  } else if (P.Lpad <= 192) RCALL(3); else RCALL(8);
#undef RCALL2
#undef RCALL
#endif
}
void launch_mg_resolve(hipStream_t st, const DevParams &P) {
  if (P.gKg == P.Kg) return;
  hipLaunchKernelGGL(k_mg_resolve, GRID1(P.gKg - P.Kg, 256), dim3(256), 0, st, P);
}
void launch_mg_mark(hipStream_t st, const DevParams &P) {
  if (P.alts == 2) hipLaunchKernelGGL(k_alt_resolve, GRID1(P.Ktot, 256), dim3(256), 0, st, P);
  hipLaunchKernelGGL(k_mg_mark, GRID1(P.Ktot, 256), dim3(256), 0, st, P);
}
void launch_ph_mark(hipStream_t st, const DevParams &P) {
  if (!P.gKg) return;
  if (P.alts == 2) hipLaunchKernelGGL(k_ph_alt_resolve, GRID1(P.gKg, 64), dim3(64), 0, st, P);
  if (P.deep_bins) hipLaunchKernelGGL(k_ph_mark, GRID1(P.gKg, MARK_BLOCK), dim3(64), 0, st, P);
  else hipLaunchKernelGGL(k_ph_mark_wide, GRID1(P.gKg, MARK_BLOCK), dim3(MARK_BLOCK), 0, st, P);
}
void launch_delay(hipStream_t st, uint32_t microseconds) { hipLaunchKernelGGL(k_delay, dim3(1), dim3(1), 0, st, microseconds); }
void launch_chain_summary(hipStream_t st, const DevParams &P, uint2 *sum, unsigned long long *tot) {
  if (P.K) hipLaunchKernelGGL(k_chain_summary, GRID1(P.K, 256), dim3(256), 0, st, P, sum, tot);
}
void launch_scatter(hipStream_t st, const DevParams &P, uint64_t cap_m, uint64_t cap_s, const uint64_t *off_m,
                    const uint64_t *off_s) {
  if (cap_m) hipLaunchKernelGGL(k_scatter_matched, GRID1(cap_m, 256), dim3(256), 0, st, P, cap_m, off_m);
  if (cap_s) hipLaunchKernelGGL(k_scatter_single, GRID1(cap_s, 256), dim3(256), 0, st, P, cap_s, off_s);
}
void launch_rec_size(hipStream_t st, const uint32_t *order, const uint16_t *lens, uint64_t cnt, uint32_t *sz) {
  if (!cnt) return;
  hipLaunchKernelGGL(k_rec_size, GRID1(cnt, 256), dim3(256), 0, st, order, lens, cnt, sz);
}
void launch_emit_dna(hipStream_t st, const uint64_t *reads, const uint16_t *lens, int S, const uint32_t *order,
                     const char *rc, uint64_t cnt, const uint64_t *off, uint32_t rec_fixed, uint8_t *dst) {
  if (!cnt) return;
  if (!off) {
    hipLaunchKernelGGL(k_emit_dna_fixed, GRID1((cnt * rec_fixed + 3) / 4, 256), dim3(256), 0, st, reads, lens, S, order, rc, cnt, rec_fixed, dst);
    return;
  }
  hipLaunchKernelGGL(k_emit_dna, GRID1(cnt, 256), dim3(256), 0, st, reads, lens, S, order, rc, cnt, off, rec_fixed, dst);
}
void launch_synth(hipStream_t st, uint8_t *dst, uint32_t n, uint32_t L, uint64_t G, uint64_t seed, uint32_t thr24) {
  if (!n) return;
  hipLaunchKernelGGL(k_synth, GRID1(n, 256), dim3(256), 0, st, dst, n, L, G, seed, thr24);
}

hipError_t sort_pairs(hipStream_t st, void *tmp, size_t &tmp_bytes, const uint64_t *kin, uint64_t *kout,
                      const uint32_t *vin, uint32_t *vout, size_t n, unsigned end_bit) {
  return rocprim::radix_sort_pairs(tmp, tmp_bytes, kin, kout, vin, vout, n, 0u, end_bit, st);
}
hipError_t sort_pairs_u32_u64(hipStream_t st, void *tmp, size_t &tmp_bytes, const uint32_t *kin, uint32_t *kout,
                              const uint64_t *vin, uint64_t *vout, size_t n, unsigned end_bit) {
  return rocprim::radix_sort_pairs(tmp, tmp_bytes, kin, kout, vin, vout, n, 0u, end_bit, st);
}
hipError_t rle(hipStream_t st, void *tmp, size_t &tmp_bytes, const uint64_t *in, size_t n, uint64_t *uniq,
               uint32_t *counts, uint32_t *nruns) {
  return rocprim::run_length_encode(tmp, tmp_bytes, in, n, uniq, counts, nruns, st);
}
hipError_t merge_by_hash(hipStream_t st, void *tmp, size_t &tmp_bytes, const uint64_t *k0, const uint64_t *k1,
                         const uint64_t *v0, const uint64_t *v1, uint64_t *kout, uint64_t *vout, size_t n0, size_t n1) {
  return rocprim::merge(tmp, tmp_bytes, k0, k1, kout, v0, v1, vout, n0, n1, rocprim::less<uint64_t>(), st);
}
hipError_t excl_scan_u32(hipStream_t st, void *tmp, size_t &tmp_bytes, const uint32_t *in, uint32_t *out, size_t n) {
  return rocprim::exclusive_scan(tmp, tmp_bytes, in, out, 0u, n, rocprim::plus<uint32_t>(), st);
}
hipError_t excl_scan_u32_to_u64(hipStream_t st, void *tmp, size_t &tmp_bytes, const uint32_t *in, uint64_t *out,
                                size_t n) {
  return rocprim::exclusive_scan(tmp, tmp_bytes, in, out, (uint64_t)0, n, rocprim::plus<uint64_t>(), st);
}

}
```

spring_amd/csrc/reorder_pipeline.cpp:

```cpp
#include <hip/hip_runtime.h>
#include <dlfcn.h>

#include <algorithm>
#include <system_error>
#include <thread>
#include <memory>
#include <atomic>
#include <chrono>
#include <cstdarg>
#include <cstdio>
#include <cstdlib>
#include <cstring>
#include <map>
#include <mutex>
#include <new>
#include <stdexcept>
#include <string>
#include <unordered_map>
#include <vector>
#include <zlib.h>

#include "reorder_device.h"
#include "reorder_internal.h"
#include "spring_reorder.h"
// ... 163 lines not shown
  if (ctx->stage != ST_FINAL) return fail(SPRING_REORDER_E_STATE, "reorder context is not finalized");
  v->dev = ctx->dev; v->st = ctx->st; v->n = ctx->n; v->L = ctx->L; v->W = ctx->W; v->S = ctx->S;
  v->reads = ctx->d_reads; v->lens = ctx->d_lens; v->nrec = ctx->nrec; v->nsing = ctx->nsing;
  v->f_order = ctx->P.f_order; v->f_order_s = ctx->P.f_order_s; v->f_rc = ctx->P.f_rc; v->f_flag = ctx->P.f_flag;
  v->f_pos = ctx->P.f_pos; v->f_len = ctx->P.f_len; v->tid_off = ctx->tid_off.data(); v->num_thr = ctx->o.num_thr;
  v->tid_off_s = ctx->tid_off_s.data();
  v->tid_mid = ctx->tid_mid.data(); v->tid_mid_s = ctx->tid_mid_s.data();
  for (int j = 0; j < 2; j++) {
    v->N_dna[j] = ctx->d_N[j]; v->N_off[j] = ctx->d_offN[j]; v->N_order[j] = ctx->d_orderN[j];
    v->N_count[j] = ctx->fq.num_reads_N[j]; v->N_bytes[j] = ctx->N_bytes[j];
  }
  v->fq_num_reads_0 = ctx->fq.num_reads[0];
  return 0;
}
hipError_t dev_alloc(int dev, size_t bytes, void **out) {
  size_t actual = 0;
  return pool_alloc(dev, bytes ? bytes : 16, out, &actual);
}
void dev_free(int dev, void *p) { if (p) pool_free(dev, p); }
}

namespace {
struct RcclId128 { char b[128]; };
struct Rccl {
  void *h = nullptr;
  int (*GetUniqueId)(void *) = nullptr;
  int (*CommInitRank)(void **, int, RcclId128, int) = nullptr;
  int (*CommDestroy)(void *) = nullptr;
  int (*CommAbort)(void *) = nullptr;
  int (*AllGather)(const void *, void *, size_t, int, void *, hipStream_t) = nullptr;
  const char *(*GetErrorString)(int) = nullptr;
};
Rccl g_rccl;
std::mutex g_rccl_mu;
int rccl_load() {
  std::lock_guard<std::mutex> lk(g_rccl_mu);
  if (g_rccl.h) return 0;
  void *h = dlopen("librccl.so.1", RTLD_NOW | RTLD_GLOBAL);
  if (!h) h = dlopen("librccl.so", RTLD_NOW | RTLD_GLOBAL);
  if (!h) return fail(SPRING_REORDER_E_HIP, "cannot load librccl.so.1: %s", dlerror());
  g_rccl.GetUniqueId = (decltype(g_rccl.GetUniqueId))dlsym(h, "ncclGetUniqueId");
  g_rccl.CommInitRank = (decltype(g_rccl.CommInitRank))dlsym(h, "ncclCommInitRank");
  g_rccl.CommDestroy = (decltype(g_rccl.CommDestroy))dlsym(h, "ncclCommDestroy");
  g_rccl.CommAbort = (decltype(g_rccl.CommAbort))dlsym(h, "ncclCommAbort");
  g_rccl.AllGather = (decltype(g_rccl.AllGather))dlsym(h, "ncclAllGather");
  g_rccl.GetErrorString = (decltype(g_rccl.GetErrorString))dlsym(h, "ncclGetErrorString");
  if (!g_rccl.GetUniqueId || !g_rccl.CommInitRank || !g_rccl.CommDestroy || !g_rccl.AllGather)
    return fail(SPRING_REORDER_E_HIP, "librccl lacks an expected entry point");
  g_rccl.h = h;
  return 0;
}
const char *rccl_err(int e) { return g_rccl.GetErrorString ? g_rccl.GetErrorString(e) : "rccl error"; }
constexpr int RCCL_UINT64 = 5;
}
#if defined(__has_include)
#if __has_include(<rccl/rccl.h>)
#include <rccl/rccl.h>
#include <type_traits>
static_assert(sizeof(ncclUniqueId) == sizeof(RcclId128) && NCCL_UNIQUE_ID_BYTES == 128, "ncclUniqueId is not 128 bytes");
static_assert((int)ncclUint64 == RCCL_UINT64, "ncclUint64 has another code");
static_assert(sizeof(ncclResult_t) == sizeof(int) && sizeof(ncclDataType_t) == sizeof(int) && sizeof(ncclComm_t) == sizeof(void *),
              "enum / handle sizes differ from the hand-written prototypes");
static_assert(std::is_same<decltype(&ncclGetUniqueId), ncclResult_t (*)(ncclUniqueId *)>::value, "ncclGetUniqueId");
static_assert(std::is_same<decltype(&ncclCommInitRank), ncclResult_t (*)(ncclComm_t *, int, ncclUniqueId, int)>::value, "ncclCommInitRank");
static_assert(std::is_same<decltype(&ncclCommDestroy), ncclResult_t (*)(ncclComm_t)>::value, "ncclCommDestroy");
static_assert(std::is_same<decltype(&ncclCommAbort), ncclResult_t (*)(ncclComm_t)>::value, "ncclCommAbort");
static_assert(std::is_same<decltype(&ncclAllGather),
                           ncclResult_t (*)(const void *, void *, size_t, ncclDataType_t, ncclComm_t, hipStream_t)>::value, "ncclAllGather");
static_assert(std::is_same<decltype(&ncclGetErrorString), const char *(*)(ncclResult_t)>::value, "ncclGetErrorString");
#endif
#endif
namespace {
}

struct spring_mg_comm {
  uint32_t rank = 0, world = 1;
  int dev = 0;
  void *rccl = nullptr;
  std::mutex mu;
  bool aborted = false;
  spring_mg_allgather_fn host_fn = nullptr;
  void *host_user = nullptr;
};

#define DMALLOC(ptr, bytes)                                   \
  do {                                                        \
    int r_ = ctx->dmalloc((void **)&(ptr), (bytes));          \
    if (r_) return r_;                                        \
  } while (0)

extern "C" {

void spring_reorder_default_opts(spring_reorder_opts *o) {
  memset(o, 0, sizeof(*o));
  o->device = -1;
  o->num_chains = 0;
  o->num_thr = 1;
}

const char *spring_reorder_last_error(void) { return g_err.c_str(); }

extern "C++" {
namespace {
struct PinCache {
  std::mutex mu;
  std::vector<void *> free_chunks;
};
PinCache g_pin;
}
namespace sr {
void *pinned_get() {
  {
    std::lock_guard<std::mutex> lk(g_pin.mu);
    if (!g_pin.free_chunks.empty()) {
      void *p = g_pin.free_chunks.back();
      g_pin.free_chunks.pop_back();
      return p;
    }
  }
  void *p = nullptr;
  if (hipHostMalloc(&p, PIN_CHUNK, hipHostMallocDefault) != hipSuccess) { (void)hipGetLastError(); return nullptr; }
  return p;
}
void pinned_put(void *p) {
  if (!p) return;
  std::lock_guard<std::mutex> lk(g_pin.mu);
  g_pin.free_chunks.push_back(p);
}
}
}

void spring_reorder_trim_pool(void) {
  {
    std::lock_guard<std::mutex> lk(g_pin.mu);
    for (void *p : g_pin.free_chunks) (void)hipHostFree(p);
    g_pin.free_chunks.clear();
  }
  for (int d = 0; d < 16; d++) {
    DevPool &p = g_pool[d];
    std::lock_guard<std::mutex> lk(p.mu);
    if (p.free_blocks.empty()) continue;
    (void)hipSetDevice(d);
    for (auto &kv : p.free_blocks) { (void)hipFree(kv.second); p.sizes.erase(kv.second); }
    p.free_blocks.clear();
    p.cached = 0;
  }
}

int spring_reorder_create(spring_reorder_ctx **out, const spring_reorder_opts *opts) {
  if (!out) return fail(SPRING_REORDER_E_ARG, "ctx is NULL");
  spring_reorder_opts o;
  if (opts) o = *opts; else spring_reorder_default_opts(&o);
  if (o.num_thr <= 0) return fail(SPRING_REORDER_E_ARG, "num_thr must be >= 1");
  int ndev = 0;
  HIPCHK(hipGetDeviceCount(&ndev));
  if (ndev <= 0) return fail(SPRING_REORDER_E_HIP, "no HIP device");
  int dev = o.device;
  if (dev < 0) HIPCHK(hipGetDevice(&dev));
  if (dev >= ndev) return fail(SPRING_REORDER_E_ARG, "device %d out of range (%d devices)", dev, ndev);
  HIPCHK(hipSetDevice(dev));
  spring_reorder_ctx *ctx = new spring_reorder_ctx();
  ctx->o = o;
  ctx->dev = dev;
  memset(&ctx->P, 0, sizeof(ctx->P));
  memset(&ctx->stats, 0, sizeof(ctx->stats));
  HIPCHK(hipStreamCreateWithFlags(&ctx->st, hipStreamNonBlocking));
  for (auto &e : ctx->ev) HIPCHK(hipEventCreate(&e));
  ctx->ev_ok = true;
  *out = ctx;
  return 0;
}

void spring_reorder_destroy(spring_reorder_ctx *ctx) {
  if (!ctx) return;
  (void)hipSetDevice(ctx->dev);
  if (ctx->st) (void)hipStreamSynchronize(ctx->st);
  if (ctx->st2) (void)hipStreamSynchronize(ctx->st2);
  if (ctx->st3) (void)hipStreamSynchronize(ctx->st3);
  for (void *p : ctx->allocs) pool_free(ctx->dev, p);
  if (ctx->ev_ok) for (auto &e : ctx->ev) (void)hipEventDestroy(e);
  if (ctx->st) (void)hipStreamDestroy(ctx->st);
  if (ctx->st2) (void)hipStreamDestroy(ctx->st2);
  if (ctx->st3) (void)hipStreamDestroy(ctx->st3);
  delete ctx;
}

static int setup_geometry(spring_reorder_ctx *ctx, uint32_t n, uint32_t max_readlen) {
  if (max_readlen == 0 || max_readlen > (uint32_t)MAX_READ_LEN)
    return fail(SPRING_REORDER_E_ARG, "Wrong bitset size. (max_readlen=%u, supported 1..511)", max_readlen);
  ctx->n = n;
  ctx->L = (int)max_readlen;
  ctx->W = (2 * ctx->L - 1) / 64 + 1;
  int S = 1;
  while (S < ctx->W) S <<= 1;
  ctx->S = S;
  ctx->Lpad = (ctx->L + 63) / 64 * 64;
  const int L = ctx->L;
  ctx->dict[0].start = L > 100 ? L / 2 - 32 : L / 2 - L * 32 / 100;
  ctx->dict[0].end = L / 2 - 1;
  ctx->dict[1].start = L / 2;
  ctx->dict[1].end = L > 100 ? L / 2 - 1 + 32 : L / 2 - 1 + L * 32 / 100;
  return 0;
}

static int unpack_on_device(spring_reorder_ctx *ctx, uint32_t *d_bad_len = nullptr) {
  if (!ctx->d_reads) DMALLOC(ctx->d_reads, (size_t)std::max<uint32_t>(ctx->n, 1) * ctx->S * sizeof(uint64_t));
  if (!ctx->d_lens) DMALLOC(ctx->d_lens, (size_t)std::max<uint32_t>(ctx->n, 1) * sizeof(uint16_t));
  HIPCHK(hipEventRecord(ctx->ev[0], ctx->st));
  const uint32_t rec = 2u + ((uint32_t)ctx->L + 3u) / 4u;
  launch_unpack(ctx->st, ctx->d_dna, ctx->d_off, ctx->n, ctx->L, ctx->W, ctx->S, rec, ctx->d_reads, ctx->d_lens, d_bad_len);
  HIPCHK(hipGetLastError());
  HIPCHK(hipEventRecord(ctx->ev[1], ctx->st));
  ctx->stage = ST_LOADED;
  return 0;
}

static int upload_chunked(spring_reorder_ctx *ctx, uint8_t *d_dst, size_t nbytes,
                          int (*fill)(void *, size_t, void *, size_t), void *self) {
  if (!nbytes) return 0;
  const size_t nchunks = (nbytes + PIN_CHUNK - 1) / PIN_CHUNK;
  const unsigned hw = std::max(1u, std::thread::hardware_concurrency());
  const int nthr = (int)std::min<size_t>(std::min<size_t>(8, hw), nchunks);
  std::atomic<size_t> next{0};
  std::atomic<int> rc{0};
  std::vector<std::string> errs((size_t)nthr);
  auto worker = [&](int ti) {
    void *pin[2] = {nullptr, nullptr};
    hipEvent_t ev[2] = {nullptr, nullptr};
    hipStream_t st = nullptr;
    bool used[2] = {false, false};
    auto bail = [&](int code, const char *what) {
      int zero = 0;
      if (rc.compare_exchange_strong(zero, code)) errs[(size_t)ti] = what;
    };
    if (hipSetDevice(ctx->dev) != hipSuccess || hipStreamCreateWithFlags(&st, hipStreamNonBlocking) != hipSuccess) {
      bail(SPRING_REORDER_E_HIP, "upload: cannot create a copy stream");
    } else {
      for (int k = 0; k < 2 && !rc.load(); k++) {
        pin[k] = pinned_get();
        if (!pin[k] || hipEventCreateWithFlags(&ev[k], hipEventDisableTiming) != hipSuccess) bail(SPRING_REORDER_E_HIP, "upload: cannot pin a staging chunk");
      }
      for (int k = 0; !rc.load(); k ^= 1) {
        const size_t i = next.fetch_add(1);
        if (i >= nchunks) break;
        const size_t off = i * PIN_CHUNK, len = std::min(PIN_CHUNK, nbytes - off);
        if (used[k] && hipEventSynchronize(ev[k]) != hipSuccess) { bail(SPRING_REORDER_E_HIP, "upload: event wait failed"); break; }
        if (fill(self, off, pin[k], len)) { bail(SPRING_REORDER_E_IO, g_err.c_str()); break; }
        if (hipMemcpyAsync(d_dst + off, pin[k], len, hipMemcpyHostToDevice, st) != hipSuccess ||
            hipEventRecord(ev[k], st) != hipSuccess) { bail(SPRING_REORDER_E_HIP, "upload: hipMemcpyAsync failed"); break; }
        used[k] = true;
      }
      (void)hipStreamSynchronize(st);
    }
    for (int k = 0; k < 2; k++) { if (ev[k]) (void)hipEventDestroy(ev[k]); pinned_put(pin[k]); }
    if (st) (void)hipStreamDestroy(st);
  };
  std::vector<std::thread> th;
  try {
    for (int t = 1; t < nthr; t++) th.emplace_back(worker, t);
  } catch (const std::system_error &) {
  }
  worker(0);
  for (auto &x : th) x.join();
  (void)hipGetLastError();
  if (rc.load()) {
    for (auto &e : errs) if (!e.empty()) return fail(rc.load(), "%s", e.c_str());
    return fail(rc.load(), "upload failed");
  }
  return 0;
}

struct D2HJob { void *dst; const void *src; size_t nbytes; };
static int download_chunked(spring_reorder_ctx *ctx, const std::vector<D2HJob> &jobs) {
  struct Piece { uint8_t *dst; const uint8_t *src; size_t len; };
  std::vector<Piece> pieces;
  for (const D2HJob &j : jobs)
    for (size_t off = 0; off < j.nbytes; off += PIN_CHUNK)
      pieces.push_back({(uint8_t *)j.dst + off, (const uint8_t *)j.src + off, std::min(PIN_CHUNK, j.nbytes - off)});
  if (pieces.empty()) return 0;
  HIPCHK(hipStreamSynchronize(ctx->st));
  const unsigned hw = std::max(1u, std::thread::hardware_concurrency());
  const int nthr = (int)std::min<size_t>(std::min<size_t>(8, hw), pieces.size());
  std::atomic<size_t> next{0};
  std::atomic<int> rc{0};
  auto worker = [&]() {
    void *pin[2] = {nullptr, nullptr};
    hipStream_t st = nullptr;
    const Piece *pending[2] = {nullptr, nullptr};
    if (hipSetDevice(ctx->dev) != hipSuccess || hipStreamCreateWithFlags(&st, hipStreamNonBlocking) != hipSuccess) rc = SPRING_REORDER_E_HIP;
    for (int k = 0; k < 2 && !rc.load(); k++) if (!(pin[k] = pinned_get())) rc = SPRING_REORDER_E_HIP;
    hipEvent_t ev[2] = {nullptr, nullptr};
    for (int k = 0; k < 2 && !rc.load(); k++) if (hipEventCreateWithFlags(&ev[k], hipEventDisableTiming) != hipSuccess) rc = SPRING_REORDER_E_HIP;
    auto drain = [&](int k) {
      if (!pending[k]) return;
      if (hipEventSynchronize(ev[k]) != hipSuccess) rc = SPRING_REORDER_E_HIP;
      else memcpy(pending[k]->dst, pin[k], pending[k]->len);
      pending[k] = nullptr;
    };
    for (int k = 0; !rc.load(); k ^= 1) {
      const size_t i = next.fetch_add(1);
      if (i >= pieces.size()) break;
      drain(k);
      if (hipMemcpyAsync(pin[k], pieces[i].src, pieces[i].len, hipMemcpyDeviceToHost, st) != hipSuccess ||
          hipEventRecord(ev[k], st) != hipSuccess) { rc = SPRING_REORDER_E_HIP; break; }
      pending[k] = &pieces[i];
      drain(k ^ 1);
// ... 336 lines not shown
  uint64_t obase = 0;
  HIPCHK(hipEventRecord(ctx->ev[6], st));
  for (int j = 0; j < 2; j++) {
    if (!f[j].nreads) continue;
    DMALLOC(ctx->d_N[j], f[j].N_bytes + 16);
    DMALLOC(ctx->d_orderN[j], (size_t)std::max<uint32_t>(f[j].n_N, 1) * 4);
    DMALLOC(ctx->d_offN[j], (size_t)std::max<uint32_t>(f[j].n_N, 1) * 8);
    ctx->N_bytes[j] = f[j].N_bytes;
    launch_pack_reads(st, f[j].d_txt, f[j].line_end, f[j].nreads, f[j].len, f[j].fclean, f[j].cidx, f[j].coff, f[j].nidx,
                      f[j].noff, cbase, obase, 0u, ctx->d_dna, ctx->d_off, ctx->d_N[j], ctx->d_orderN[j], ctx->d_offN[j]);
    HIPCHK(hipGetLastError());
    cbase += f[j].n_clean; obase += f[j].clean_bytes; rbase += (uint32_t)f[j].nreads;
  }
  (void)rbase;
  ctx->uniform = n_clean > 0 && std::min(f[0].min_clean, f[1].min_clean) == maxlen;
  if (ctx->uniform) { ctx->dfree(ctx->d_off); ctx->d_off = nullptr; }
  r = unpack_on_device(ctx);
  if (r) return r;
  HIPCHK(hipEventRecord(ctx->ev[7], st));
  HIPCHK(hipStreamSynchronize(st));
  { float ms = 0; if (hipEventElapsedTime(&ms, ctx->ev[6], ctx->ev[7]) == hipSuccess) ctx->fq_ms += ms; }
  ms_dev = ctx->fq_ms;
  ctx->fq.ms_device = ms_dev;
  if (info) info->ms_device = ms_dev;
  for (int j = 0; j < 2; j++) {
    ctx->dfree(f[j].d_txt); ctx->dfree(f[j].line_end); ctx->dfree(f[j].len); ctx->dfree(f[j].fclean); ctx->dfree(f[j].szc);
    ctx->dfree(f[j].fN); ctx->dfree(f[j].szN); ctx->dfree(f[j].cidx); ctx->dfree(f[j].nidx); ctx->dfree(f[j].coff);
    ctx->dfree(f[j].noff);
  }
  ctx->dfree(d_err);
  return 0;
}

int spring_reorder_fastq_N(spring_reorder_ctx *ctx, int32_t which, uint8_t *n_dna, size_t cap, size_t *nbytes,
                           uint32_t *order_N, uint32_t *count) {
  if (!ctx || ctx->stage < ST_LOADED) return fail(SPRING_REORDER_E_STATE, "fastq_N: load_fastq first");
  if (which < 0 || which > 1) return fail(SPRING_REORDER_E_ARG, "which must be 0 or 1");
  HIPCHK(hipSetDevice(ctx->dev));
  const uint32_t nN = ctx->fq.num_reads_N[which];
  if (nbytes) *nbytes = ctx->N_bytes[which];
  if (count) *count = nN;
  if (n_dna && ctx->N_bytes[which]) {
    if (cap < ctx->N_bytes[which]) return fail(SPRING_REORDER_E_ARG, "fastq_N: buffer too small");
    HIPCHK(hipMemcpy(n_dna, ctx->d_N[which], ctx->N_bytes[which], hipMemcpyDeviceToHost));
  }
  if (order_N && nN) HIPCHK(hipMemcpy(order_N, ctx->d_orderN[which], (size_t)nN * 4, hipMemcpyDeviceToHost));
  return 0;
}

size_t spring_synth_dna_bytes(uint32_t n, uint32_t L) { return (size_t)n * (2u + (L + 3u) / 4u); }

int spring_synth_dna_host(uint8_t *dst, uint32_t n, uint32_t L, uint64_t G, uint64_t seed, uint32_t err_ppm) {
  if (L == 0 || L > (uint32_t)MAX_READ_LEN || G < L) return fail(SPRING_REORDER_E_ARG, "bad synth geometry");
  if ((err_ppm & SYN_PAIRED_FLAG) && (n & 1)) return fail(SPRING_REORDER_E_ARG, "a paired pool holds an even number of reads");
  const uint32_t rec = 2u + (L + 3u) / 4u, thr = syn_err_thr24(err_ppm);
  for (uint64_t i = 0; i < n; i++) {
    uint8_t *o = dst + i * rec;
    uint64_t pos; uint32_t rc;
    syn_read_params(seed, G, L, i, (err_ppm & SYN_PAIRED_FLAG) ? n / 2 : 0, &pos, &rc);
    o[0] = (uint8_t)(L & 0xff); o[1] = (uint8_t)(L >> 8);
    for (uint32_t b = 0; b < (L + 3) / 4; b++) {
      uint32_t v = 0;
      for (uint32_t q = 0; q < 4; q++) {
        uint32_t j = 4 * b + q;
        if (j < L) v |= syn_nat_to_spring(syn_read_base(seed, G, L, thr, i, j, pos, rc)) << (2 * q);
      }
      o[2 + b] = (uint8_t)v;
    }
  }
  return 0;
}

int spring_synth_genome_host(uint8_t *dst, uint64_t G, uint64_t seed, uint32_t flags) {
  if (!dst) return fail(SPRING_REORDER_E_ARG, "dst is NULL");
  for (uint64_t p = 0; p < G; p++) {
    uint64_t gp = p;
    if (flags & SYN_REPEAT_FLAG) {
      const uint64_t seg = G / 8, k = seg ? gp / seg : 0;
      if (seg && k < 8 && (k & 1) == 0) gp %= seg;
    }
    dst[p] = (uint8_t)"ACGT"[(flags & SYN_GENOMIC_FLAG) ? syn_genomic_base(seed, gp) : syn_genome_base(seed, gp)];
  }
  return 0;
}

int spring_synth_dna_device(void *d_dst, uint32_t n, uint32_t L, uint64_t G, uint64_t seed, uint32_t err_ppm) {
  if (!d_dst || L == 0 || L > (uint32_t)MAX_READ_LEN || G < L) return fail(SPRING_REORDER_E_ARG, "bad synth arguments");
  if ((err_ppm & SYN_PAIRED_FLAG) && (n & 1)) return fail(SPRING_REORDER_E_ARG, "a paired pool holds an even number of reads");
  launch_synth(nullptr, (uint8_t *)d_dst, n, L, G, seed, syn_err_thr24(err_ppm));
  HIPCHK(hipGetLastError());
  HIPCHK(hipStreamSynchronize(nullptr));
  return 0;
}

int spring_reorder_load_synth(spring_reorder_ctx *ctx, uint32_t n, uint32_t L, uint64_t G, uint64_t seed,
                              uint32_t err_ppm) {
  if (!ctx) return fail(SPRING_REORDER_E_ARG, "ctx is NULL");
  if (ctx->stage != ST_CREATED) return fail(SPRING_REORDER_E_STATE, "load_synth: context already loaded");
  if (L == 0 || L > (uint32_t)MAX_READ_LEN || G < L) return fail(SPRING_REORDER_E_ARG, "bad synth geometry");
  if ((err_ppm & SYN_PAIRED_FLAG) && (n & 1)) return fail(SPRING_REORDER_E_ARG, "a paired pool holds an even number of reads");
  HIPCHK(hipSetDevice(ctx->dev));
  int r = setup_geometry(ctx, n, L);
  if (r) return r;
  ctx->uniform = true;
  ctx->dna_bytes = spring_synth_dna_bytes(n, L);
  DMALLOC(ctx->d_dna, ctx->dna_bytes + 16);
  launch_synth(ctx->st, ctx->d_dna, n, L, G, seed, syn_err_thr24(err_ppm));
  HIPCHK(hipGetLastError());
  return unpack_on_device(ctx);
}

int spring_reorder_download_dna(spring_reorder_ctx *ctx, uint8_t *dst, size_t cap) {
  if (!ctx || ctx->stage < ST_LOADED) return fail(SPRING_REORDER_E_STATE, "download_dna: nothing loaded");
  if (cap < ctx->dna_bytes) return fail(SPRING_REORDER_E_ARG, "buffer too small");
  HIPCHK(hipSetDevice(ctx->dev));
  HIPCHK(hipStreamSynchronize(ctx->st));
  if (ctx->dna_bytes) HIPCHK(hipMemcpy(dst, ctx->d_dna, ctx->dna_bytes, hipMemcpyDeviceToHost));
  return 0;
}

int spring_reorder_download_reads(spring_reorder_ctx *ctx, uint64_t *limbs, uint16_t *len) {
  if (!ctx || ctx->stage < ST_LOADED) return fail(SPRING_REORDER_E_STATE, "download_reads: nothing loaded");
  HIPCHK(hipSetDevice(ctx->dev));
  HIPCHK(hipStreamSynchronize(ctx->st));
  if (!ctx->n) return 0;
  if (limbs)
    HIPCHK(hipMemcpy2D(limbs, (size_t)ctx->W * 8, ctx->d_reads, (size_t)ctx->S * 8, (size_t)ctx->W * 8, ctx->n,
                       hipMemcpyDeviceToHost));
  if (len) HIPCHK(hipMemcpy(len, ctx->d_lens, (size_t)ctx->n * 2, hipMemcpyDeviceToHost));
  return 0;
}

static uint64_t pow2ceil(uint64_t x) {
  uint64_t p = 1;
  while (p < x) p <<= 1;
  return p;
}

static double now_ms() {
  return std::chrono::duration<double, std::milli>(std::chrono::steady_clock::now().time_since_epoch()).count();
}
#define DBG_T(label)                                                                         \
  do {                                                                                       \
    if (dbg) { (void)hipStreamSynchronize(st); double t_ = now_ms(); fprintf(stderr, "[dict] %-14s %8.2f ms\n", label, t_ - t_last); t_last = t_; } \
  } while (0)

static TabView tab_view(const spring_reorder_ctx *ctx) {
  TabView t;
  t.buck = ctx->fpt;
  t.bshift = ctx->bshift; t.minz = ctx->minz; t.lshift = ctx->lshift;
  return t;
}

int spring_reorder_build_dict(spring_reorder_ctx *ctx) {
  double t_last = now_ms();
  if (!ctx) return fail(SPRING_REORDER_E_ARG, "ctx is NULL");
  const bool dbg = ctx->o.debug != 0;
  if (ctx->stage != ST_LOADED) return fail(SPRING_REORDER_E_STATE, "build_dict: load reads first");
  HIPCHK(hipSetDevice(ctx->dev));
  hipStream_t st = ctx->st;
  const uint32_t n = ctx->n;
  HIPCHK(hipEventRecord(ctx->ev[2], st));
  uint64_t *uhash[2] = {nullptr, nullptr};
  uint32_t *ustart[2] = {nullptr, nullptr}, *ucount[2] = {nullptr, nullptr};
  for (int l = 0; l < 2; l++) {
    DictDev &d = ctx->dict[l];
    uint32_t m = 0;
    uint32_t *d_slot = nullptr, *d_flag = nullptr;
    void *d_tmp = nullptr;
    size_t tmp_bytes = 0;
    if (n) {
      if (ctx->uniform) {
        m = ctx->L > d.end ? n : 0;
      } else {
        DMALLOC(d_flag, (size_t)n * 4);
        DMALLOC(d_slot, (size_t)n * 4);
        launch_flag_in_dict(st, ctx->d_lens, n, d.end, d_flag);
        HIPCHK(excl_scan_u32(st, nullptr, tmp_bytes, d_flag, d_slot, n));
        DMALLOC(d_tmp, tmp_bytes);
        HIPCHK(excl_scan_u32(st, d_tmp, tmp_bytes, d_flag, d_slot, n));
        uint32_t last_slot = 0, last_flag = 0;
        HIPCHK(hipMemcpyAsync(&last_slot, d_slot + (n - 1), 4, hipMemcpyDeviceToHost, st));
        HIPCHK(hipMemcpyAsync(&last_flag, d_flag + (n - 1), 4, hipMemcpyDeviceToHost, st));
        HIPCHK(hipStreamSynchronize(st));
        m = last_slot + last_flag;
        ctx->dfree(d_tmp); d_tmp = nullptr;
      }
    }
    d.numreads = m;
    d.numkeys = 0;
    d.ndeep = 0; d.big_reads = 0; d.mid_reads = 0;
    if (m == 0) {
      DMALLOC(d.urec, 16);
      DMALLOC(d.ids, 16);
      DMALLOC(d.deep, 16);
      DMALLOC(d.d_ndeep, 16);
      HIPCHK(hipMemsetAsync(d.d_ndeep, 0, 12, st));
      if (d_flag) { ctx->dfree(d_flag); ctx->dfree(d_slot); }
      continue;
    }
    uint64_t *k_in = nullptr, *k_out = nullptr;
    uint32_t *v_in = nullptr, *cnt = nullptr, *d_nruns = nullptr;
    DMALLOC(k_in, (size_t)m * 8);
    DMALLOC(k_out, (size_t)m * 8);
    DMALLOC(v_in, (size_t)m * 4);
    DMALLOC(d.ids, (size_t)m * 4);
    DBG_T("alloc keys");
    launch_keys(st, ctx->d_reads, ctx->d_lens, ctx->uniform ? nullptr : d_slot, n, ctx->S, d.start, d.end, k_in, v_in);
    HIPCHK(hipGetLastError());
    DBG_T("k_keys");
    const unsigned end_bit = 64;
    tmp_bytes = 0;
    HIPCHK(sort_pairs(st, nullptr, tmp_bytes, k_in, k_out, v_in, d.ids, m, end_bit));
    DMALLOC(d_tmp, tmp_bytes);
    HIPCHK(sort_pairs(st, d_tmp, tmp_bytes, k_in, k_out, v_in, d.ids, m, end_bit));
    DBG_T("sort");
    ctx->dfree(d_tmp); d_tmp = nullptr;
    ctx->dfree(v_in);
    DMALLOC(cnt, (size_t)m * 4);
    DMALLOC(d_nruns, 16);
    tmp_bytes = 0;
    HIPCHK(rle(st, nullptr, tmp_bytes, k_out, m, k_in, cnt, d_nruns));
    DMALLOC(d_tmp, tmp_bytes);
    HIPCHK(rle(st, d_tmp, tmp_bytes, k_out, m, k_in, cnt, d_nruns));
    uint32_t numkeys = 0;
    HIPCHK(hipMemcpyAsync(&numkeys, d_nruns, 4, hipMemcpyDeviceToHost, st));
    HIPCHK(hipStreamSynchronize(st));
    ctx->dfree(d_tmp); d_tmp = nullptr;
    ctx->dfree(k_out); ctx->dfree(d_nruns);
    d.numkeys = numkeys;
    DBG_T("rle");
    DMALLOC(ustart[l], (size_t)numkeys * 4);
    tmp_bytes = 0;
    HIPCHK(excl_scan_u32(st, nullptr, tmp_bytes, cnt, ustart[l], numkeys));
    DMALLOC(d_tmp, tmp_bytes);
    HIPCHK(excl_scan_u32(st, d_tmp, tmp_bytes, cnt, ustart[l], numkeys));
    DBG_T("scan");
    uhash[l] = k_in;
    ucount[l] = cnt;
    DMALLOC(d.urec, (size_t)numkeys * 16);
    DMALLOC(d.deep, ((size_t)m / DEEP_BIN + 1) * 4);
    DMALLOC(d.d_ndeep, 16);
    HIPCHK(hipMemsetAsync(d.d_ndeep, 0, 12, st));
    HIPCHK(hipStreamSynchronize(st));
    ctx->dfree(d_tmp);
    if (d_flag) { ctx->dfree(d_flag); ctx->dfree(d_slot); }
  }
  const uint64_t nk0 = ctx->dict[0].numkeys, nk1 = ctx->dict[1].numkeys, nm = nk0 + nk1;
  const int tab_scale = ctx->o.tab_scale > 0 ? ctx->o.tab_scale : 2;
  const uint64_t nb = std::max<uint64_t>(8, pow2ceil(std::max<uint64_t>(2, (nm * 10 + 15) / 16)) * (uint64_t)pow2ceil(tab_scale));
  ctx->bshift = 64;
  for (uint64_t v = nb; v > 1; v >>= 1) ctx->bshift--;
  ctx->minz = (ctx->dict[0].end - ctx->dict[0].start + 1 == MINZ_WL && ctx->L <= 192 && ctx->o.table_mode == 2) ? 1 : 0;
  ctx->lshift = 32 - (64 - ctx->bshift - 2);
  if (ctx->lshift < 1) return fail(SPRING_REORDER_E_ARG, "build_dict: table too large for minimizer addressing");
  ctx->stats.table_minz = ctx->minz; ctx->stats.table_marked_lines = 0;
  DMALLOC(ctx->fpt, nb * 32);
  HIPCHK(hipMemsetAsync(ctx->fpt, 0, nb * 32, st));
  uint32_t *const tab_words = reinterpret_cast<uint32_t *>(ctx->fpt);
  DBG_T("alloc+memset tab");
  if (nm) {
    uint64_t *mv0 = nullptr, *mv1 = nullptr, *mh = nullptr, *mv = nullptr;
    void *d_tmp = nullptr;
    DMALLOC(mv0, std::max<uint64_t>(nk0, 1) * 8);
    DMALLOC(mv1, std::max<uint64_t>(nk1, 1) * 8);
    launch_iota_tag(st, mv0, nk0, 0ull);
    launch_iota_tag(st, mv1, nk1, 1ull << 63);
    const uint64_t *h_in = nullptr, *v_in = nullptr;
    if (nk0 && nk1) {
      DMALLOC(mh, nm * 8);
      DMALLOC(mv, nm * 8);
      size_t tb = 0;
      HIPCHK(merge_by_hash(st, nullptr, tb, uhash[0], uhash[1], mv0, mv1, mh, mv, nk0, nk1));
      DMALLOC(d_tmp, tb);
      HIPCHK(merge_by_hash(st, d_tmp, tb, uhash[0], uhash[1], mv0, mv1, mh, mv, nk0, nk1));
      h_in = mh; v_in = mv;
    } else {
      h_in = nk0 ? uhash[0] : uhash[1];
      v_in = nk0 ? mv0 : mv1;
    }
    DBG_T("merge");
    DictBuild db[2];
    for (int l = 0; l < 2; l++) {
      DictDev &d = ctx->dict[l];
      db[l].ustart = ustart[l]; db[l].ucount = ucount[l]; db[l].ids = d.ids; db[l].urec = d.urec;
      db[l].deep = d.deep; db[l].ndeep = d.d_ndeep;
    }
    uint32_t *bk_in = nullptr, *bk_out = nullptr, *d_marked = nullptr;
    uint64_t *tp_in = nullptr, *tp_out = nullptr;
    ctx->marked_lines = 0;
    void *d_tmp2 = nullptr;
    if (!ctx->minz) {
      launch_tab_insert(st, h_in, v_in, nm, db[0], db[1], tab_words, ctx->bshift);
    } else {
      DMALLOC(bk_in, nm * 4); DMALLOC(bk_out, nm * 4);
      DMALLOC(tp_in, nm * 8); DMALLOC(tp_out, nm * 8);
      launch_minz_prepare(st, h_in, v_in, nm, db[0], db[1], ctx->lshift, bk_in, tp_in);
      DBG_T("minz prepare");
      const unsigned end_bit = (unsigned)(64 - ctx->bshift);
      size_t tb = 0;
      HIPCHK(sort_pairs_u32_u64(st, nullptr, tb, bk_in, bk_out, tp_in, tp_out, nm, end_bit));
      DMALLOC(d_tmp2, tb);
      HIPCHK(sort_pairs_u32_u64(st, d_tmp2, tb, bk_in, bk_out, tp_in, tp_out, nm, end_bit));
      DBG_T("minz sort");
      DMALLOC(d_marked, 16);
      HIPCHK(hipMemsetAsync(d_marked, 0, 4, st));
      launch_tab_insert_minz(st, bk_out, tp_out, nm, tab_words, ctx->bshift, d_marked);
      HIPCHK(hipMemcpyAsync(&ctx->marked_lines, d_marked, 4, hipMemcpyDeviceToHost, st));
    }
    HIPCHK(hipGetLastError());
    uint32_t nd[2][3] = {{0, 0, 0}, {0, 0, 0}};
    for (int l = 0; l < 2; l++)
      HIPCHK(hipMemcpyAsync(nd[l], ctx->dict[l].d_ndeep, 12, hipMemcpyDeviceToHost, st));
    HIPCHK(hipStreamSynchronize(st));
    for (int l = 0; l < 2; l++) { ctx->dict[l].ndeep = nd[l][0]; ctx->dict[l].big_reads = nd[l][1]; ctx->dict[l].mid_reads = nd[l][2]; }
    if (dbg) fprintf(stderr, "[dict] reads %u + %u, keys %u + %u, bins >= %u: %u + %u, reads in bins >= %u: %u + %u, >= %u: %u + %u\n",
                     ctx->dict[0].numreads, ctx->dict[1].numreads, ctx->dict[0].numkeys, ctx->dict[1].numkeys, DEEP_BIN, nd[0][0], nd[1][0],
                     MID_BIN, nd[0][2], nd[1][2], BIG_BIN, nd[0][1], nd[1][1]);
    ctx->stats.table_marked_lines = ctx->marked_lines;
    DBG_T("insert");
    ctx->dfree(mv0); ctx->dfree(mv1); ctx->dfree(mh); ctx->dfree(mv); ctx->dfree(d_tmp);
    ctx->dfree(bk_in); ctx->dfree(bk_out); ctx->dfree(tp_in); ctx->dfree(tp_out); ctx->dfree(d_tmp2); ctx->dfree(d_marked);
  }
  for (int l = 0; l < 2; l++) { ctx->dfree(uhash[l]); ctx->dfree(ustart[l]); ctx->dfree(ucount[l]); }
  DBG_T("free temps");
  HIPCHK(hipEventRecord(ctx->ev[3], st));
  ctx->stage = ST_DICT;
  return 0;
}

int spring_reorder_dict_lookup(spring_reorder_ctx *ctx, int32_t which, const uint64_t *keys, uint32_t nkeys,
                               uint32_t *bin_size, uint32_t *bin_ids, size_t ids_cap) {
  if (!ctx || ctx->stage < ST_DICT) return fail(SPRING_REORDER_E_STATE, "dict_lookup: build_dict first");
  if (which < 0 || which > 1) return fail(SPRING_REORDER_E_ARG, "which must be 0 or 1");
  HIPCHK(hipSetDevice(ctx->dev));
  DictDev &d = ctx->dict[which];
  uint64_t *dk = nullptr;
  uint32_t *ds = nullptr, *dc = nullptr;
  DMALLOC(dk, (size_t)nkeys * 8);
  DMALLOC(ds, (size_t)nkeys * 4);
  DMALLOC(dc, (size_t)nkeys * 4);
  std::vector<uint32_t> hs(nkeys), hc(nkeys), hids(d.numreads);
  if (nkeys) {
    HIPCHK(hipMemcpyAsync(dk, keys, (size_t)nkeys * 8, hipMemcpyHostToDevice, ctx->st));
    launch_dict_lookup(ctx->st, tab_view(ctx), d.urec, which, ctx->d_reads, ctx->S, d.start, d.end, dk, nkeys, ds, dc);
    HIPCHK(hipMemcpyAsync(hs.data(), ds, (size_t)nkeys * 4, hipMemcpyDeviceToHost, ctx->st));
    HIPCHK(hipMemcpyAsync(hc.data(), dc, (size_t)nkeys * 4, hipMemcpyDeviceToHost, ctx->st));
  }
  if (d.numreads) HIPCHK(hipMemcpyAsync(hids.data(), d.ids, (size_t)d.numreads * 4, hipMemcpyDeviceToHost, ctx->st));
  HIPCHK(hipStreamSynchronize(ctx->st));
  ctx->dfree(dk); ctx->dfree(ds); ctx->dfree(dc);
  size_t o = 0;
  for (uint32_t i = 0; i < nkeys; i++) {
    if (hc[i] != 0xffffffffu && (hc[i] & 0x80000000u)) {
      bin_size[i] = 1;
      if (o + 1 > ids_cap) return fail(SPRING_REORDER_E_ARG, "bin_ids too small");
      bin_ids[o++] = hs[i];
      continue;
    }
    bin_size[i] = hc[i];
    if (hc[i] == 0xffffffffu) continue;
    if (o + hc[i] > ids_cap) return fail(SPRING_REORDER_E_ARG, "bin_ids too small");
    memcpy(bin_ids + o, hids.data() + hs[i], (size_t)hc[i] * 4);
    o += hc[i];
  }
  return 0;
}

static bool dict_is_deep(const spring_reorder_ctx *ctx) {
  const uint64_t nd = (uint64_t)ctx->dict[0].numreads + ctx->dict[1].numreads, nk = (uint64_t)ctx->dict[0].numkeys + ctx->dict[1].numkeys;
  return nd * 10 >= nk * 13;
}
static bool dict_has_heavy_tail(const spring_reorder_ctx *ctx) {
  const uint64_t mid = (uint64_t)ctx->dict[0].mid_reads + ctx->dict[1].mid_reads, nd = (uint64_t)ctx->dict[0].numreads + ctx->dict[1].numreads;
  return nd > 0 && mid * 1000 >= nd;
}
static bool dict_is_contended(const spring_reorder_ctx *ctx) {
  const uint64_t mid = (uint64_t)ctx->dict[0].mid_reads + ctx->dict[1].mid_reads, nd = (uint64_t)ctx->dict[0].numreads + ctx->dict[1].numreads;
  return nd > 0 && mid * 4 >= nd;
}
static bool dict_wants_deep_kernel(const spring_reorder_ctx *ctx) {
  const uint64_t nd = (uint64_t)ctx->dict[0].numreads + ctx->dict[1].numreads, nk = (uint64_t)ctx->dict[0].numkeys + ctx->dict[1].numkeys;
  return nd * 100 >= nk * 115 || dict_has_heavy_tail(ctx);
}
static bool dict_is_very_deep(const spring_reorder_ctx *ctx) {
  const uint64_t big = (uint64_t)ctx->dict[0].big_reads + ctx->dict[1].big_reads, nd = (uint64_t)ctx->dict[0].numreads + ctx->dict[1].numreads;
  return dict_is_deep(ctx) && nd > 0 && big * 4 >= nd;
}
static void fill_params(spring_reorder_ctx *ctx, DevParams &P) {
  const spring_reorder_opts &o = ctx->o;
  P.reads = ctx->d_reads; P.lens = ctx->d_lens; P.n = ctx->n;
  P.L = ctx->L; P.W = ctx->W; P.S = ctx->S; P.Lpad = ctx->Lpad;
  P.maxshift = ctx->L / 2;
  memset(P.plan, 0, sizeof(P.plan));
  if (o.first_shifts < 0) { P.plan[0][0] = 4; P.plan[0][1] = 4; P.plan[0][2] = 8; P.plan[0][3] = 8; }
  else if (o.first_shifts > 0) { P.plan[0][0] = std::min(16, o.first_shifts); P.plan[0][1] = 16; }
  else if (o.fused >= 0 && o.fused != 2 && !o.collect_stats && !o.force_literal_update) {
    P.plan[0][0] = 4; P.plan[0][1] = 8; P.plan[0][2] = 16;
  } else { P.plan[0][0] = 8; P.plan[0][1] = 16; }
  P.plan[1][0] = 16; P.plan[1][1] = 16;
  bool user_plan[2] = {false, false};
  for (int w = 0; w < 2; w++) {
    const int32_t *up = w ? o.plan1 : o.plan0;
    if (up[0] <= 0) continue;
    int k = 0, sum = 0;
    int tmp[6] = {0, 0, 0, 0, 0, 0};
    for (; k < 6 && up[k] > 0; k++) {
      if (up[k] > 16 || sum + up[k] > 32) break;
      tmp[k] = up[k]; sum += up[k];
    }
    if (k == 0) continue;
    memcpy(P.plan[w], tmp, sizeof(tmp));
    user_plan[w] = true;
  }
  ctx->user_plan0 = user_plan[0];
  P.seed_wide = o.seed_wide < 0 ? 0 : 1;
  P.search_wpb = (o.search_wpb == 1 || o.search_wpb == 2 || o.search_wpb == 4) ? o.search_wpb : 1;
  P.dbg_search_lds = std::max(0, o.dbg_search_lds);
  P.dbg_apply_lds = std::max(0, o.dbg_apply_lds);
  P.uniform_len = ctx->uniform ? 1 : 0;
  P.wl = ctx->dict[0].end - ctx->dict[0].start + 1;
  for (int l = 0; l < 2; l++) {
    P.dstart[l] = ctx->dict[l].start; P.dend[l] = ctx->dict[l].end; P.numkeys[l] = ctx->dict[l].numkeys;
    P.urec[l] = ctx->dict[l].urec; P.ids[l] = ctx->dict[l].ids;
    P.epos[l] = nullptr;
  }
  P.idmask = 0xffffffffu;
  P.tab = tab_view(ctx);
  P.deep_bins = o.deep_bins ? (o.deep_bins > 0) : dict_wants_deep_kernel(ctx);
  if (o.alternatives == 2) P.deep_bins = 1;
  if (P.deep_bins && !dict_is_deep(ctx) && o.first_shifts == 0 && !user_plan[0]) {
    memset(P.plan[0], 0, sizeof(P.plan[0]));
    P.plan[0][0] = 8; P.plan[0][1] = 16;
  }
  if (P.deep_bins && dict_is_deep(ctx) && o.first_shifts == 0 && o.fused >= 0 && !o.collect_stats && !o.force_literal_update &&
      !user_plan[0]) {
    memset(P.plan[0], 0, sizeof(P.plan[0]));
    P.plan[0][0] = 2; P.plan[0][1] = 6; P.plan[0][2] = 8; P.plan[0][3] = 16;
    if (!user_plan[1]) {
      memset(P.plan[1], 0, sizeof(P.plan[1]));
      P.plan[1][0] = 4; P.plan[1][1] = 12; P.plan[1][2] = 16;
    }
  }
  const bool very_deep = P.deep_bins && (dict_is_very_deep(ctx) || (dict_has_heavy_tail(ctx) && !dict_is_deep(ctx)));
  P.long_budget = o.long_budget < 0 ? 0 : (o.long_budget ? o.long_budget : (very_deep ? 8 : 0));
  P.long_blocks = 256;
  P.long_min = P.long_budget < 8 ? 0 : 512;
  if (o.long_min > 0) P.long_min = o.long_min;
  if (o.long_blocks > 0) P.long_blocks = o.long_blocks;
  P.long_part = o.long_split > 0 ? o.long_split : (o.long_split < 0 ? 0 : 192);
  P.longq = nullptr;
  P.lctl = nullptr; P.lparts = nullptr; P.lhead = nullptr; P.lbin = nullptr; P.lbcode = nullptr; P.lbin_stride = 0;
  P.sig[0] = P.sig[1] = nullptr;
}
static uint32_t auto_chains(uint32_t n, bool deep, bool very_deep, bool heavy_tail = false) {
  uint64_t k = (deep || heavy_tail) ? n >> 7 : n >> 10;
  const uint64_t cap = ((deep && !very_deep) || (heavy_tail && !deep)) ? 131072 : 65536;
  if (k < 1) k = 1;
  if (k > cap) k = cap;
  if (k >= 16384) k &= ~2047ull;
  return (uint32_t)k;
}

static int setup_chains(spring_reorder_ctx *ctx, uint32_t K, uint32_t c0, uint32_t Ktot, bool fused, void *d_prop,
                        bool allow_phases = false) {
  hipStream_t st = ctx->st;
  const uint32_t n = ctx->n;
  ctx->K = K;
  DevParams &P = ctx->P;
  fill_params(ctx, P);
  const uint64_t nublk = std::max<uint64_t>(((uint64_t)n + (1u << UBLK_SHIFT) - 1) >> UBLK_SHIFT, 1);
  const uint64_t nwords = nublk << (UBLK_SHIFT - 6);
  const size_t nn = std::max<uint32_t>(n, 1);
  if (ctx->o.alternatives > 2) return fail(SPRING_REORDER_E_ARG, "alternatives: <= 0 (library's choice), 1 or 2");
  if (ctx->o.phases > 2) return fail(SPRING_REORDER_E_ARG, "phases: <= 0 (library's choice), 1 or 2");
// ... 1203 lines not shown
```

spring_amd/reorder.py:

```python
import ctypes as C
from dataclasses import dataclass

import numpy as np

from . import _lib


class ReorderError(RuntimeError):
    """Raised where the reference throws std::runtime_error (call_template_functions.cpp:60)."""


@dataclass
class ReorderOpts:
    device: int = -1
    num_chains: int = 0
    num_thr: int = 1
    collect_stats: bool = False
    time_search: bool = False
    force_literal_update: bool = False
    rounds_per_sync: int = 0
    first_shifts: int = 0
    seed_wide: int = 0
    tab_scale: int = 0
    search_wpb: int = 0
    dbg_search_lds: int = 0
    dbg_apply_lds: int = 0
    fused: int = 0
    deep_bins: int = 0
    long_budget: int = 0
    devices: tuple = ()
    mg_host_transport: bool = False
    plan0: tuple = ()
    plan1: tuple = ()
    long_min: int = 0
    long_blocks: int = 0
    entry_flags: int = 0
    long_split: int = 0
    debug: bool = False
    out_writers: int = 0
    alternatives: int = 0
    table_mode: int = 0
    phases: int = 0
    known_absent: int = 0

    def to_c(self):
        o = _lib.Opts()
        _lib.lib().spring_reorder_default_opts(C.byref(o))
        o.device, o.num_chains, o.num_thr = self.device, self.num_chains, self.num_thr
        o.collect_stats, o.time_search = int(self.collect_stats), int(self.time_search)
        o.force_literal_update, o.rounds_per_sync = int(self.force_literal_update), self.rounds_per_sync
        o.first_shifts, o.seed_wide, o.tab_scale = self.first_shifts, self.seed_wide, self.tab_scale
        o.search_wpb, o.dbg_search_lds, o.dbg_apply_lds = self.search_wpb, self.dbg_search_lds, self.dbg_apply_lds
        o.fused, o.deep_bins = self.fused, self.deep_bins
        o.long_budget = self.long_budget
        if len(self.devices) > 8:
            raise ValueError("at most 8 devices")
        o.table_mode = self.table_mode
        for i, v in enumerate(tuple(self.plan0)[:6]):
            o.plan0[i] = int(v)
        for i, v in enumerate(tuple(self.plan1)[:6]):
            o.plan1[i] = int(v)
        o.long_min, o.long_blocks, o.debug = self.long_min, self.long_blocks, int(self.debug)
        o.long_split, o.entry_flags = self.long_split, self.entry_flags
        o.out_writers = self.out_writers
        o.alternatives = self.alternatives
        o.phases = self.phases
        o.known_absent = self.known_absent
        o.num_devices = len(self.devices)
        for i, d in enumerate(self.devices):
            o.devices[i] = d
        o.mg_host_transport = int(self.mg_host_transport)
        return o


def _chk(rc):
    if rc != 0:
        raise ReorderError("%s (code %d)" % (_lib.lib().spring_reorder_last_error().decode(), rc))


class ReorderStage:

    def __init__(self, opts: ReorderOpts = None):
        self.opts = opts or ReorderOpts()
        self._L = _lib.lib()
        self._h = C.c_void_p()
        _chk(self._L.spring_reorder_create(C.byref(self._h), C.byref(self.opts.to_c())))
        self.n = 0
        self.max_readlen = 0

    def close(self):
        if self._h:
            self._L.spring_reorder_destroy(self._h)
            self._h = C.c_void_p()

    def __enter__(self):
        return self

    def __exit__(self, *a):
        self.close()

    def __del__(self):
        try:
            self.close()
        except Exception:
            pass

    def load_dna(self, dna: bytes, n: int, max_readlen: int):
        buf = np.frombuffer(dna, dtype=np.uint8)
        _chk(self._L.spring_reorder_load_dna(self._h, buf.ctypes.data if len(buf) else None, len(buf), n,
                                             max_readlen))
        self.n, self.max_readlen = n, max_readlen

    def load_dna_device(self, dptr: int, nbytes: int, n: int, max_readlen: int, fixed_len: bool):
        _chk(self._L.spring_reorder_load_dna_device(self._h, C.c_void_p(dptr), nbytes, n, max_readlen,
                                                    int(fixed_len)))
        self.n, self.max_readlen = n, max_readlen

    def load_synth(self, n, L, G, seed, err_ppm=10000):
        _chk(self._L.spring_reorder_load_synth(self._h, n, L, G, seed, err_ppm))
        self.n, self.max_readlen = n, L

    def load_fastq(self, fastq_1: bytes, fastq_2: bytes = None):
        a = np.frombuffer(fastq_1, dtype=np.uint8)
        b = np.frombuffer(fastq_2, dtype=np.uint8) if fastq_2 is not None else None
        info = _lib.FastqInfo()
        _chk(self._L.spring_reorder_load_fastq(
            self._h, a.ctypes.data if len(a) else None, len(a),
            (b.ctypes.data if len(b) else C.c_void_p(1)) if b is not None else None, len(b) if b is not None else 0,
            C.byref(info)))
        self.n = info.num_reads_clean[0] + info.num_reads_clean[1]
        self.max_readlen = max(int(info.max_readlen), 1)
        return dict(num_reads=list(info.num_reads), num_reads_clean=list(info.num_reads_clean),
                    num_reads_N=list(info.num_reads_N), max_readlen=int(info.max_readlen),
                    ms_device=float(info.ms_device))

    def fastq_N(self, which=0):
        nb, cnt = C.c_size_t(), C.c_uint32()
        _chk(self._L.spring_reorder_fastq_N(self._h, which, None, 0, C.byref(nb), None, C.byref(cnt)))
        buf = np.zeros(max(nb.value, 1), np.uint8)
        order = np.zeros(max(cnt.value, 1), np.uint32)
        _chk(self._L.spring_reorder_fastq_N(self._h, which, buf.ctypes.data, nb.value, C.byref(nb), order.ctypes.data,
                                            C.byref(cnt)))
        return buf[:nb.value].tobytes(), order[:cnt.value]

    def build_dict(self):
        _chk(self._L.spring_reorder_build_dict(self._h))

    def run_chains(self):
        _chk(self._L.spring_reorder_run_chains(self._h))

    def auto_chains(self):
        k, d = C.c_uint32(0), C.c_int32(0)
        _chk(self._L.spring_reorder_auto_chains(self._h, C.byref(k), C.byref(d)))
        return k.value, bool(d.value)

    def finalize(self):
        _chk(self._L.spring_reorder_finalize(self._h))

    def run(self):
        self.build_dict()
        self.run_chains()
        self.finalize()
        return self

    def stats(self):
        s = _lib.Stats()
        _chk(self._L.spring_reorder_get_stats(self._h, C.byref(s)))
        return s.asdict()

    def streams(self):
        st = self.stats()
        nm, ns, T = st["n_matched"], st["n_single"], self.opts.num_thr
        out = dict(order=np.zeros(max(nm, 1), np.uint32), rc=np.zeros(max(nm, 1), np.uint8),
                   flag=np.zeros(max(nm, 1), np.uint8), pos=np.zeros(max(nm, 1), np.int64),
                   rlen=np.zeros(max(nm, 1), np.uint16), order_s=np.zeros(max(ns, 1), np.uint32),
                   tid_off=np.zeros(T + 1, np.uint64), tid_off_s=np.zeros(T + 1, np.uint64))
        _chk(self._L.spring_reorder_download(self._h, *[out[k].ctypes.data for k in (
            "order", "rc", "flag", "pos", "rlen", "order_s", "tid_off", "tid_off_s")]))
        for k in ("order", "rc", "flag", "pos", "rlen"):
            out[k] = out[k][:nm]
        out["order_s"] = out["order_s"][:ns]
        out["tid_mid"], out["tid_mid_s"] = np.zeros(T, np.uint64), np.zeros(T, np.uint64)
        _chk(self._L.spring_reorder_tid_split(self._h, out["tid_mid"].ctypes.data, out["tid_mid_s"].ctypes.data))
        out["stats"] = st
        return out

    def emit_dna(self, tid: int) -> bytes:
        nb = C.c_size_t()
        _chk(self._L.spring_reorder_emit_dna(self._h, tid, None, 0, C.byref(nb)))
        buf = np.zeros(max(nb.value, 1), np.uint8)
        _chk(self._L.spring_reorder_emit_dna(self._h, tid, buf.ctypes.data, nb.value, C.byref(nb)))
        return buf[:nb.value].tobytes()

    def dict_lookup(self, which, keys):
        keys = np.ascontiguousarray(keys, dtype=np.uint64)
        sizes = np.zeros(max(len(keys), 1), np.uint32)
        ids = np.zeros(max(self.n, 1) * 2, np.uint32)
        _chk(self._L.spring_reorder_dict_lookup(self._h, which, keys.ctypes.data, len(keys), sizes.ctypes.data,
                                                ids.ctypes.data, len(ids)))
        return sizes[:len(keys)], ids

    def download_reads(self):
        W = (2 * self.max_readlen - 1) // 64 + 1
        limbs = np.zeros((max(self.n, 1), W), np.uint64)
        ln = np.zeros(max(self.n, 1), np.uint16)
        _chk(self._L.spring_reorder_download_reads(self._h, limbs.ctypes.data, ln.ctypes.data))
        return limbs[:self.n], ln[:self.n]

    def download_dna(self) -> bytes:
        nb = self._L.spring_synth_dna_bytes(self.n, self.max_readlen)
        buf = np.zeros(max(nb, 1), np.uint8)
        _chk(self._L.spring_reorder_download_dna(self._h, buf.ctypes.data, nb))
        p = 0
        for _ in range(self.n):
            p += 2 + ((int(buf[p]) | (int(buf[p + 1]) << 8)) + 3) // 4
        return buf[:p].tobytes()


def reorder_dna(dna: bytes, n: int, max_readlen: int, opts: ReorderOpts = None):
    with ReorderStage(opts) as s:
# ... 41 lines not shown
```

Baseline: 324.6 Mreads/s.

## Speed up dictionary build: prefix radix sort with repair, fused keys, staged unpack

Replaces the full 64-bit key radix sort in the dictionary build with a sort on only the top 40 or 48 bits. A repair pass then finds runs with equal prefixes but different keys and re-sorts them in LDS, falling back to a full sort if a run is too long or the list overflows. It also adds an LDS-staged unpack kernel for fixed-length records and computes both dictionaries' keys in one kernel. The merge now tags values internally instead of building iota arrays, and the overflow table-insert pass is compacted through an index list. These add host syncs and extra kernels, and the repair path could be slower when many prefix collisions occur.

```diff
diff --git a/include/spring_reorder.h b/include/spring_reorder.h
--- a/include/spring_reorder.h
+++ b/include/spring_reorder.h
@@ -47,6 +47,7 @@
   int32_t alternatives;
   int32_t phases;
   int32_t known_absent;
+  int32_t sort_prefix_bits;
 } spring_reorder_opts;
 
 typedef struct {
@@ -67,6 +68,11 @@
   uint64_t alternatives;
   uint64_t phases;
   double ms_search_busy;
+  uint64_t sort_prefix_bits;
+  uint64_t sort_repaired_runs;
+  uint64_t sort_full_sorts;
+  uint64_t sort_long_runs;
+  uint64_t sort_list_overflows;
 } spring_reorder_stats;
 
 void spring_reorder_default_opts(spring_reorder_opts *o);
diff --git a/spring_amd/_lib.py b/spring_amd/_lib.py
--- a/spring_amd/_lib.py
+++ b/spring_amd/_lib.py
@@ -46,7 +46,8 @@
                 ("num_devices", C.c_int32), ("devices", C.c_int32 * 8), ("mg_host_transport", C.c_int32),
                 ("table_mode", C.c_int32), ("plan0", C.c_int32 * 6), ("plan1", C.c_int32 * 6), ("long_min", C.c_int32),
                 ("long_blocks", C.c_int32), ("debug", C.c_int32), ("long_split", C.c_int32), ("entry_flags", C.c_int32),
-                ("out_writers", C.c_int32), ("alternatives", C.c_int32), ("phases", C.c_int32), ("known_absent", C.c_int32)]
+                ("out_writers", C.c_int32), ("alternatives", C.c_int32), ("phases", C.c_int32), ("known_absent", C.c_int32),
+                ("sort_prefix_bits", C.c_int32)]
 
 
 class FastqInfo(C.Structure):
@@ -105,7 +106,9 @@
                    ("ms_exchange", C.c_double), ("ms_resolve_mark", C.c_double), ("chains", C.c_uint64),
                    ("deep_pool", C.c_uint64), ("long_searches", C.c_uint64),
                    ("table_minz", C.c_uint64), ("table_marked_lines", C.c_uint64), ("long_splits", C.c_uint64), ("alternatives", C.c_uint64), ("phases", C.c_uint64),
-                   ("ms_search_busy", C.c_double)])
+                   ("ms_search_busy", C.c_double),
+                   ("sort_prefix_bits", C.c_uint64), ("sort_repaired_runs", C.c_uint64), ("sort_full_sorts", C.c_uint64),
+                   ("sort_long_runs", C.c_uint64), ("sort_list_overflows", C.c_uint64)])
 
     def asdict(self):
         d = {}
diff --git a/spring_amd/csrc/reorder_device.h b/spring_amd/csrc/reorder_device.h
--- a/spring_amd/csrc/reorder_device.h
+++ b/spring_amd/csrc/reorder_device.h
@@ -157,18 +157,26 @@
   uint32_t *f_order; char *f_rc; char *f_flag; long long *f_pos; uint16_t *f_len; uint32_t *f_order_s;
 };
 
+constexpr int UNPACK_READS = 128;
 void launch_unpack(hipStream_t st, const uint8_t *dna, const uint64_t *off, uint32_t n, int L, int W, int S,
                    uint32_t rec_fixed, uint64_t *reads, uint16_t *lens, uint32_t *bad_len = nullptr);
 void launch_flag_in_dict(hipStream_t st, const uint16_t *lens, uint32_t n, int dend, uint32_t *flag);
 void launch_keys(hipStream_t st, const uint64_t *reads, const uint16_t *lens, const uint32_t *slot, uint32_t n,
                  int S, int dstart, int dend, uint64_t *keys, uint32_t *vals);
+void launch_keys2(hipStream_t st, const uint64_t *reads, uint32_t n, int S, int dstart0, int dend0, int dstart1, int dend1,
+                  uint64_t *keys0, uint32_t *vals0, uint64_t *keys1, uint32_t *vals1);
+constexpr int SORT_FIX_MAX = 1024;
+void launch_sort_repair(hipStream_t st, uint64_t *k, uint32_t *ids, uint64_t m, unsigned prefix_bits, uint32_t *list,
+                        uint32_t cap, uint32_t *ctr, uint2 *runs);
 struct DictBuild {
   const uint32_t *ustart, *ucount, *ids;
   ulonglong2 *urec;
   uint32_t *deep, *ndeep;
 };
 void launch_tab_insert(hipStream_t st, const uint64_t *mhash, const uint64_t *mval, uint64_t nmerged, DictBuild d0,
-                       DictBuild d1, uint32_t *fpt, int bshift);
+                       DictBuild d1, uint32_t *fpt, int bshift, uint32_t *ovf);
+void launch_tab_overflow(hipStream_t st, const uint64_t *mhash, const uint64_t *mval, uint64_t nmerged, DictBuild d0,
+                         DictBuild d1, uint32_t *fpt, int bshift, uint32_t *ovf, uint32_t novf);
 void launch_minz_prepare(hipStream_t st, const uint64_t *mhash, const uint64_t *mval, uint64_t nmerged, DictBuild d0,
                          DictBuild d1, int lshift, uint32_t *bucket, uint64_t *tagpay);
 void launch_tab_insert_minz(hipStream_t st, const uint32_t *bucket_sorted, const uint64_t *tagpay_sorted, uint64_t nmerged,
@@ -176,7 +184,7 @@
 hipError_t sort_pairs_u32_u64(hipStream_t st, void *tmp, size_t &tmp_bytes, const uint32_t *kin, uint32_t *kout,
                               const uint64_t *vin, uint64_t *vout, size_t n, unsigned end_bit);
 hipError_t merge_by_hash(hipStream_t st, void *tmp, size_t &tmp_bytes, const uint64_t *k0, const uint64_t *k1,
-                         const uint64_t *v0, const uint64_t *v1, uint64_t *kout, uint64_t *vout, size_t n0, size_t n1);
+                         uint64_t tag1, uint64_t *kout, uint64_t *vout, size_t n0, size_t n1);
 void launch_iota_tag(hipStream_t st, uint64_t *v, uint64_t n, uint64_t tag);
 void launch_build_epos(hipStream_t st, const uint32_t *ids, uint64_t m, uint32_t *epos);
 void launch_trim_bins(hipStream_t st, const uint32_t *deep, const uint32_t *ndeep, uint32_t ndeep_host,
@@ -219,7 +227,7 @@
 hipError_t reduce_min_u32(hipStream_t st, void *tmp, size_t &tmp_bytes, const uint32_t *in, uint32_t *out, size_t n);
 
 hipError_t sort_pairs(hipStream_t st, void *tmp, size_t &tmp_bytes, const uint64_t *kin, uint64_t *kout,
-                      const uint32_t *vin, uint32_t *vout, size_t n, unsigned end_bit);
+                      const uint32_t *vin, uint32_t *vout, size_t n, unsigned end_bit, unsigned begin_bit = 0);
 hipError_t rle(hipStream_t st, void *tmp, size_t &tmp_bytes, const uint64_t *in, size_t n, uint64_t *uniq,
                uint32_t *counts, uint32_t *nruns);
 hipError_t excl_scan_u32(hipStream_t st, void *tmp, size_t &tmp_bytes, const uint32_t *in, uint32_t *out, size_t n);
diff --git a/spring_amd/csrc/reorder_kernels.hip b/spring_amd/csrc/reorder_kernels.hip
--- a/spring_amd/csrc/reorder_kernels.hip
+++ b/spring_amd/csrc/reorder_kernels.hip
@@ -207,6 +207,58 @@
   reads[i * S + j] = v;
 }
 
+__global__ __launch_bounds__(256) void k_unpack_fixed(const uint8_t *__restrict__ dna, uint32_t n, int L, int W, int lgS,
+                                                      uint32_t rec, uint64_t *__restrict__ reads,
+                                                      uint16_t *__restrict__ lens, uint32_t *__restrict__ bad_len) {
+  extern __shared__ uint4 s_unpack[];
+  const uint32_t r0 = blockIdx.x * (uint32_t)UNPACK_READS;
+  const uint32_t nr = min((uint32_t)UNPACK_READS, n - r0);
+  const uint8_t *g = dna + (uint64_t)r0 * rec;
+  const uint32_t sh = (uint32_t)((uintptr_t)g & 15u);
+  const uint4 *ga = reinterpret_cast<const uint4 *>(g - sh);
+  const uint32_t nchunk = (sh + nr * rec + 15u) >> 4;
+  for (uint32_t k = threadIdx.x; k < nchunk; k += 256) s_unpack[k] = ga[k];
+  __syncthreads();
+  const uint8_t *sb = reinterpret_cast<const uint8_t *>(s_unpack);
+  const uint32_t *sw = reinterpret_cast<const uint32_t *>(s_unpack);
+  const bool chk = bad_len != nullptr;
+  auto len_of = [&](uint32_t r) -> uint32_t {
+    const uint32_t p = sh + r * rec;
+    return (uint32_t)sb[p] | ((uint32_t)sb[p + 1] << 8);
+  };
+  auto limb = [&](uint32_t m) -> uint64_t {
+    const uint32_t r = m >> lgS, j = m & ((1u << lgS) - 1u);
+    if ((int)j >= W) return 0;
+    uint32_t len = len_of(r);
+    if (chk && len != (uint32_t)L) len = (uint32_t)L;
+    const uint32_t nb = min((len + 3u) / 4u, rec - 2u), pos = 8u * j;
+    if (pos >= nb) return 0;
+    const uint32_t p = sh + r * rec + 2u + pos, k = p >> 2, s8 = (p & 3u) * 8u;
+    uint64_t v = (uint64_t)sw[k] | ((uint64_t)sw[k + 1] << 32);
+    if (s8) v = (v >> s8) | ((uint64_t)sw[k + 2] << (64u - s8));
+    if (nb - pos < 8u) v &= (1ull << (8u * (nb - pos))) - 1ull;
+    return v;
+  };
+  for (uint32_t t = threadIdx.x; 2u * t < nr; t += 256) {
+    const uint32_t r = 2u * t;
+    uint32_t l0 = len_of(r), l1 = r + 1 < nr ? len_of(r + 1) : (uint32_t)L;
+    if (chk && (l0 != (uint32_t)L || l1 != (uint32_t)L)) {
+      *bad_len = 1u;
+      l0 = l1 = (uint32_t)L;
+    }
+    if (r + 1 < nr) *reinterpret_cast<uint32_t *>(lens + r0 + r) = l0 | (l1 << 16);
+    else lens[r0 + r] = (uint16_t)l0;
+  }
+  const uint32_t nl = nr << lgS;
+  uint64_t *out = reads + ((uint64_t)r0 << lgS);
+  for (uint32_t q = threadIdx.x; 2u * q < nl; q += 256) {
+    const uint32_t m = 2u * q;
+    const uint64_t v0 = limb(m);
+    if (m + 1 < nl) *reinterpret_cast<ulonglong2 *>(out + m) = make_ulonglong2(v0, limb(m + 1));
+    else out[m] = v0;
+  }
+}
+
 __global__ void k_flag_in_dict(const uint16_t *__restrict__ lens, uint32_t n, int dend,
                                uint32_t *__restrict__ flag) {
   uint32_t i = blockIdx.x * blockDim.x + threadIdx.x;
@@ -229,17 +281,110 @@
   keys[o] = mix64(v);
   vals[o] = i;
 }
+__global__ void k_keys2(const uint64_t *__restrict__ reads, uint32_t n, int S, int dstart0, int klen0, int dstart1,
+                        int klen1, uint64_t *__restrict__ keys0, uint32_t *__restrict__ vals0,
+                        uint64_t *__restrict__ keys1, uint32_t *__restrict__ vals1) {
+  uint32_t i = blockIdx.x * blockDim.x + threadIdx.x;
+  if (i >= n) return;
+  const uint64_t *r = reads + (uint64_t)i * S;
+  keys0[i] = mix64(read_window(r, S, dstart0, 2 * klen0));
+  vals0[i] = i;
+  keys1[i] = mix64(read_window(r, S, dstart1, 2 * klen1));
+  vals1[i] = i;
+}
+
+__global__ void k_sort_breaks(const uint64_t *__restrict__ k, uint64_t m, int shift, uint32_t *__restrict__ list,
+                              uint32_t cap, uint32_t *__restrict__ ctr) {
+  const uint64_t i = (uint64_t)blockIdx.x * blockDim.x + threadIdx.x;
+  if (i == 0 || i >= m) return;
+  const uint64_t a = k[i - 1], b = k[i];
+  if (a != b && (a >> shift) == (b >> shift)) {
+    const uint32_t s = atomicAdd(ctr, 1u);
+    if (s < cap) list[s] = (uint32_t)i;
+  }
+}
+__global__ __launch_bounds__(256) void k_sort_runs(const uint64_t *__restrict__ k, uint64_t m, int shift,
+                                                   const uint32_t *__restrict__ list, uint32_t cap,
+                                                   uint32_t *__restrict__ ctr, uint2 *__restrict__ runs) {
+  const uint32_t nbr = ctr[0];
+  if (nbr > cap) return;
+  const uint32_t lane = threadIdx.x & 63u, nwaves = gridDim.x * 4u;
+  for (uint32_t c = blockIdx.x * 4u + (threadIdx.x >> 6); c < nbr; c += nwaves) {
+    const uint64_t i = list[c];
+    const uint64_t p = k[i] >> shift, prev = k[i - 1];
+    uint64_t s = 0, e = 0;
+    bool mine = true;
+    for (uint64_t w = 2;; w += 64) {
+      const uint64_t o = w + lane;
+      const bool valid = o <= i;
+      const uint64_t v = valid ? k[i - o] : 0;
+      const bool inrun = valid && (v >> shift) == p;
+      const unsigned long long m_out = __ballot(!inrun), m_dif = __ballot(inrun && v != prev);
+      const int f_out = m_out ? __ffsll(m_out) - 1 : 64, f_dif = m_dif ? __ffsll(m_dif) - 1 : 64;
+      if (f_dif < f_out) { mine = false; break; }
+      if (f_out < 64) { s = i - (w + (uint64_t)f_out) + 1; break; }
+      if (w + 64 > (uint64_t)SORT_FIX_MAX) {
+        if (lane == 0) atomicOr(ctr + 2, 1u);
+        mine = false;
+        break;
+      }
+    }
+    if (!mine) continue;
+    for (uint64_t w = i + 1;; w += 64) {
+      const uint64_t x = w + lane;
+      const bool inrun = x < m && (k[x] >> shift) == p;
+      const unsigned long long m_out = __ballot(!inrun);
+      if (m_out) { e = w + (uint64_t)(__ffsll(m_out) - 1); break; }
+      if (w + 64 - s > (uint64_t)SORT_FIX_MAX) { e = w + 64; break; }
+    }
+    if (e - s > (uint64_t)SORT_FIX_MAX) {
+      if (lane == 0) atomicOr(ctr + 2, 1u);
+      continue;
+    }
+    if (lane == 0) runs[atomicAdd(ctr + 1, 1u)] = make_uint2((uint32_t)s, (uint32_t)(e - s));
+  }
+}
+__global__ __launch_bounds__(64) void k_sort_fix(uint64_t *__restrict__ k, uint32_t *__restrict__ ids, uint32_t cap,
+                                                 const uint32_t *__restrict__ ctr, const uint2 *__restrict__ runs) {
+  __shared__ uint64_t sk[SORT_FIX_MAX];
+  __shared__ uint32_t sv[SORT_FIX_MAX];
+  if (ctr[0] > cap || ctr[2]) return;
+  const uint32_t nruns = ctr[1];
+  for (uint32_t c = blockIdx.x; c < nruns; c += gridDim.x) {
+    const uint2 rn = runs[c];
+    for (uint32_t x = threadIdx.x; x < rn.y; x += 64) { sk[x] = k[(uint64_t)rn.x + x]; sv[x] = ids[(uint64_t)rn.x + x]; }
+    __syncthreads();
+    for (uint32_t x = threadIdx.x; x < rn.y; x += 64) {
+      const uint64_t h = sk[x];
+      uint32_t rank = 0;
+      for (uint32_t y = 0; y < rn.y; y++) rank += (sk[y] < h || (sk[y] == h && y < x)) ? 1u : 0u;
+      k[(uint64_t)rn.x + rank] = h;
+      ids[(uint64_t)rn.x + rank] = sv[x];
+    }
+    __syncthreads();
+  }
+}
 
 template <bool OVERFLOW>
 __global__ void k_tab_insert(const uint64_t *__restrict__ mhash, const uint64_t *__restrict__ mval, uint64_t nm,
-                             DictBuild d0, DictBuild d1, uint32_t *fpt, int bshift) {
-  const uint64_t i = (uint64_t)blockIdx.x * blockDim.x + threadIdx.x;
-  if (i >= nm) return;
+                             DictBuild d0, DictBuild d1, uint32_t *fpt, int bshift, uint32_t *ovf) {
+  uint64_t i = (uint64_t)blockIdx.x * blockDim.x + threadIdx.x;
+  int rank = 4;
+  if (OVERFLOW) {
+    if (i >= ovf[0]) return;
+    i = ovf[1 + i];
+  } else {
+    if (i >= nm) return;
+    const uint64_t bi = bucket_of(mhash[i], bshift);
+    rank = 0;
+    while (rank < 4 && i > (uint64_t)rank && bucket_of(mhash[i - 1 - rank], bshift) == bi) rank++;
+    if (rank >= 4) {
+      ovf[1 + atomicAdd(ovf, 1u)] = (uint32_t)i;
+      return;
+    }
+  }
   const uint64_t h = mhash[i];
   const uint64_t b0 = bucket_of(h, bshift);
-  int rank = 0;
-  while (rank < 4 && i > (uint64_t)rank && bucket_of(mhash[i - 1 - rank], bshift) == b0) rank++;
-  if (OVERFLOW != (rank >= 4)) return;
   const uint64_t mv = mval[i];
   const uint32_t l = (uint32_t)(mv >> 63), u = (uint32_t)mv;
   const DictBuild &d = l ? d1 : d0;
@@ -2623,6 +2768,13 @@
 void launch_unpack(hipStream_t st, const uint8_t *dna, const uint64_t *off, uint32_t n, int L, int W, int S,
                    uint32_t rec_fixed, uint64_t *reads, uint16_t *lens, uint32_t *bad_len) {
   if (!n) return;
+  if (!off && !((uintptr_t)reads & 15u) && !((uintptr_t)lens & 3u)) {
+    int lgS = 0;
+    while ((1 << lgS) < S) lgS++;
+    const size_t lds = ((size_t)UNPACK_READS * rec_fixed + 15 + 12 + 15) / 16 * 16;
+    hipLaunchKernelGGL(k_unpack_fixed, GRID1(n, UNPACK_READS), dim3(256), lds, st, dna, n, L, W, lgS, rec_fixed, reads, lens, bad_len);
+    return;
+  }
   uint64_t tot = (uint64_t)n * S;
   hipLaunchKernelGGL(k_unpack, GRID1(tot, 256), dim3(256), 0, st, dna, off, n, L, W, S, rec_fixed, reads, lens, bad_len);
 }
@@ -2633,11 +2785,27 @@
                  int S, int dstart, int dend, uint64_t *keys, uint32_t *vals) {
   hipLaunchKernelGGL(k_keys, GRID1(n, 256), dim3(256), 0, st, reads, lens, slot, n, S, dstart, dend, keys, vals);
 }
+void launch_keys2(hipStream_t st, const uint64_t *reads, uint32_t n, int S, int dstart0, int dend0, int dstart1, int dend1,
+                  uint64_t *keys0, uint32_t *vals0, uint64_t *keys1, uint32_t *vals1) {
+  hipLaunchKernelGGL(k_keys2, GRID1(n, 256), dim3(256), 0, st, reads, n, S, dstart0, dend0 - dstart0 + 1, dstart1,
+                     dend1 - dstart1 + 1, keys0, vals0, keys1, vals1);
+}
+void launch_sort_repair(hipStream_t st, uint64_t *k, uint32_t *ids, uint64_t m, unsigned prefix_bits, uint32_t *list,
+                        uint32_t cap, uint32_t *ctr, uint2 *runs) {
+  const int shift = 64 - (int)prefix_bits;
+  hipLaunchKernelGGL(k_sort_breaks, GRID1(m, 256), dim3(256), 0, st, k, m, shift, list, cap, ctr);
+  hipLaunchKernelGGL(k_sort_runs, dim3(1024), dim3(256), 0, st, k, m, shift, list, cap, ctr, runs);
+  hipLaunchKernelGGL(k_sort_fix, dim3(4096), dim3(64), 0, st, k, ids, cap, ctr, runs);
+}
 void launch_tab_insert(hipStream_t st, const uint64_t *mhash, const uint64_t *mval, uint64_t nmerged, DictBuild d0,
-                       DictBuild d1, uint32_t *fpt, int bshift) {
+                       DictBuild d1, uint32_t *fpt, int bshift, uint32_t *ovf) {
   if (!nmerged) return;
-  hipLaunchKernelGGL(k_tab_insert<false>, GRID1(nmerged, 256), dim3(256), 0, st, mhash, mval, nmerged, d0, d1, fpt, bshift);
-  hipLaunchKernelGGL(k_tab_insert<true>, GRID1(nmerged, 256), dim3(256), 0, st, mhash, mval, nmerged, d0, d1, fpt, bshift);
+  hipLaunchKernelGGL(k_tab_insert<false>, GRID1(nmerged, 256), dim3(256), 0, st, mhash, mval, nmerged, d0, d1, fpt, bshift, ovf);
+}
+void launch_tab_overflow(hipStream_t st, const uint64_t *mhash, const uint64_t *mval, uint64_t nmerged, DictBuild d0,
+                         DictBuild d1, uint32_t *fpt, int bshift, uint32_t *ovf, uint32_t novf) {
+  if (!novf) return;
+  hipLaunchKernelGGL(k_tab_insert<true>, GRID1(novf, 256), dim3(256), 0, st, mhash, mval, nmerged, d0, d1, fpt, bshift, ovf);
 }
 void launch_minz_prepare(hipStream_t st, const uint64_t *mhash, const uint64_t *mval, uint64_t nmerged, DictBuild d0,
                          DictBuild d1, int lshift, uint32_t *bucket, uint64_t *tagpay) {
@@ -2830,8 +2998,11 @@
 }
 
 hipError_t sort_pairs(hipStream_t st, void *tmp, size_t &tmp_bytes, const uint64_t *kin, uint64_t *kout,
-                      const uint32_t *vin, uint32_t *vout, size_t n, unsigned end_bit) {
-  return rocprim::radix_sort_pairs(tmp, tmp_bytes, kin, kout, vin, vout, n, 0u, end_bit, st);
+                      const uint32_t *vin, uint32_t *vout, size_t n, unsigned end_bit, unsigned begin_bit) {
+  if (begin_bit != 0)
+    return rocprim::radix_sort_pairs<rocprim::radix_sort_config<rocprim::default_config, rocprim::default_config, rocprim::default_config, 0>>(
+        tmp, tmp_bytes, kin, kout, vin, vout, n, begin_bit, end_bit, st);
+  return rocprim::radix_sort_pairs(tmp, tmp_bytes, kin, kout, vin, vout, n, begin_bit, end_bit, st);
 }
 hipError_t sort_pairs_u32_u64(hipStream_t st, void *tmp, size_t &tmp_bytes, const uint32_t *kin, uint32_t *kout,
                               const uint64_t *vin, uint64_t *vout, size_t n, unsigned end_bit) {
@@ -2842,8 +3013,9 @@
   return rocprim::run_length_encode(tmp, tmp_bytes, in, n, uniq, counts, nruns, st);
 }
 hipError_t merge_by_hash(hipStream_t st, void *tmp, size_t &tmp_bytes, const uint64_t *k0, const uint64_t *k1,
-                         const uint64_t *v0, const uint64_t *v1, uint64_t *kout, uint64_t *vout, size_t n0, size_t n1) {
-  return rocprim::merge(tmp, tmp_bytes, k0, k1, kout, v0, v1, vout, n0, n1, rocprim::less<uint64_t>(), st);
+                         uint64_t tag1, uint64_t *kout, uint64_t *vout, size_t n0, size_t n1) {
+  return rocprim::merge(tmp, tmp_bytes, k0, k1, kout, rocprim::counting_iterator<uint64_t>(0),
+                        rocprim::counting_iterator<uint64_t>(tag1), vout, n0, n1, rocprim::less<uint64_t>(), st);
 }
 hipError_t excl_scan_u32(hipStream_t st, void *tmp, size_t &tmp_bytes, const uint32_t *in, uint32_t *out, size_t n) {
   return rocprim::exclusive_scan(tmp, tmp_bytes, in, out, 0u, n, rocprim::plus<uint32_t>(), st);
diff --git a/spring_amd/csrc/reorder_pipeline.cpp b/spring_amd/csrc/reorder_pipeline.cpp
--- a/spring_amd/csrc/reorder_pipeline.cpp
+++ b/spring_amd/csrc/reorder_pipeline.cpp
@@ -339,6 +339,8 @@
   spring_reorder_opts o;
   if (opts) o = *opts; else spring_reorder_default_opts(&o);
   if (o.num_thr <= 0) return fail(SPRING_REORDER_E_ARG, "num_thr must be >= 1");
+  if (o.sort_prefix_bits < 0 || o.sort_prefix_bits > 64)
+    return fail(SPRING_REORDER_E_ARG, "sort_prefix_bits: 0 (library's choice) or 1 .. 64 bits of the key hash (64 = the full sort)");
   int ndev = 0;
   HIPCHK(hipGetDeviceCount(&ndev));
   if (ndev <= 0) return fail(SPRING_REORDER_E_HIP, "no HIP device");
@@ -981,6 +983,8 @@
   return t;
 }
 
+static unsigned sort_prefix_auto(uint64_t m) { return m <= (1ull << 29) ? 40u : 48u; }
+
 int spring_reorder_build_dict(spring_reorder_ctx *ctx) {
   double t_last = now_ms();
   if (!ctx) return fail(SPRING_REORDER_E_ARG, "ctx is NULL");
@@ -992,6 +996,11 @@
   HIPCHK(hipEventRecord(ctx->ev[2], st));
   uint64_t *uhash[2] = {nullptr, nullptr};
   uint32_t *ustart[2] = {nullptr, nullptr}, *ucount[2] = {nullptr, nullptr};
+  const bool both_dense = n && ctx->uniform && ctx->L > ctx->dict[0].end && ctx->L > ctx->dict[1].end;
+  uint64_t *keys_both[2] = {nullptr, nullptr};
+  uint32_t *vals_both[2] = {nullptr, nullptr};
+  ctx->stats.sort_repaired_runs = 0; ctx->stats.sort_full_sorts = 0; ctx->stats.sort_prefix_bits = 0;
+  ctx->stats.sort_long_runs = 0; ctx->stats.sort_list_overflows = 0;
   for (int l = 0; l < 2; l++) {
     DictDev &d = ctx->dict[l];
     uint32_t m = 0;
@@ -1028,22 +1037,64 @@
       if (d_flag) { ctx->dfree(d_flag); ctx->dfree(d_slot); }
       continue;
     }
-    uint64_t *k_in = nullptr, *k_out = nullptr;
-    uint32_t *v_in = nullptr, *cnt = nullptr, *d_nruns = nullptr;
-    DMALLOC(k_in, (size_t)m * 8);
+    uint64_t *k_in = keys_both[l], *k_out = nullptr;
+    uint32_t *v_in = vals_both[l], *cnt = nullptr, *d_nruns = nullptr;
+    if (!k_in) {
+      DMALLOC(k_in, (size_t)m * 8);
+      DMALLOC(v_in, (size_t)m * 4);
+    }
     DMALLOC(k_out, (size_t)m * 8);
-    DMALLOC(v_in, (size_t)m * 4);
     DMALLOC(d.ids, (size_t)m * 4);
     DBG_T("alloc keys");
-    launch_keys(st, ctx->d_reads, ctx->d_lens, ctx->uniform ? nullptr : d_slot, n, ctx->S, d.start, d.end, k_in, v_in);
+    if (l == 0 && both_dense) {
+      DMALLOC(keys_both[1], (size_t)n * 8);
+      DMALLOC(vals_both[1], (size_t)n * 4);
+      launch_keys2(st, ctx->d_reads, n, ctx->S, d.start, d.end, ctx->dict[1].start, ctx->dict[1].end, k_in, v_in,
+                   keys_both[1], vals_both[1]);
+    } else if (!keys_both[l]) {
+      launch_keys(st, ctx->d_reads, ctx->d_lens, ctx->uniform ? nullptr : d_slot, n, ctx->S, d.start, d.end, k_in, v_in);
+    }
     HIPCHK(hipGetLastError());
     DBG_T("k_keys");
-    const unsigned end_bit = 64;
-    tmp_bytes = 0;
-    HIPCHK(sort_pairs(st, nullptr, tmp_bytes, k_in, k_out, v_in, d.ids, m, end_bit));
-    DMALLOC(d_tmp, tmp_bytes);
-    HIPCHK(sort_pairs(st, d_tmp, tmp_bytes, k_in, k_out, v_in, d.ids, m, end_bit));
-    DBG_T("sort");
+    const unsigned T = ctx->o.sort_prefix_bits > 0 ? (unsigned)ctx->o.sort_prefix_bits : sort_prefix_auto(m);
+    ctx->stats.sort_prefix_bits = T;
+    bool full = T >= 64;
+    if (!full) {
+      uint32_t *d_ctr = nullptr, *d_list = nullptr;
+      uint2 *d_runs = nullptr;
+      const uint32_t cap = m / 4 + 1024;
+      DMALLOC(d_ctr, 16);
+      DMALLOC(d_list, (size_t)cap * 4);
+      DMALLOC(d_runs, (size_t)cap * 8);
+      HIPCHK(hipMemsetAsync(d_ctr, 0, 16, st));
+      tmp_bytes = 0;
+      HIPCHK(sort_pairs(st, nullptr, tmp_bytes, k_in, k_out, v_in, d.ids, m, 64, 64 - T));
+      DMALLOC(d_tmp, tmp_bytes);
+      HIPCHK(sort_pairs(st, d_tmp, tmp_bytes, k_in, k_out, v_in, d.ids, m, 64, 64 - T));
+      DBG_T("prefix sort");
+      launch_sort_repair(st, k_out, d.ids, m, T, d_list, cap, d_ctr, d_runs);
+      HIPCHK(hipGetLastError());
+      uint32_t ctr[4] = {0, 0, 0, 0};
+      HIPCHK(hipMemcpyAsync(ctr, d_ctr, 16, hipMemcpyDeviceToHost, st));
+      HIPCHK(hipStreamSynchronize(st));
+      full = ctr[0] > cap || ctr[2] != 0;
+      if (ctr[0] > cap) ctx->stats.sort_list_overflows++;
+      else if (ctr[2]) ctx->stats.sort_long_runs++;
+      if (!full) ctx->stats.sort_repaired_runs += ctr[1];
+      if (dbg) fprintf(stderr, "[dict] prefix bits %u: %u hash changes inside runs, %u runs re-ordered%s\n", T, ctr[0], ctr[1],
+                       full ? " -- not repairable in place: full sort" : "");
+      ctx->dfree(d_tmp); d_tmp = nullptr;
+      ctx->dfree(d_ctr); ctx->dfree(d_list); ctx->dfree(d_runs);
+      DBG_T("sort repair");
+    }
+    if (full) {
+      if (T < 64) ctx->stats.sort_full_sorts++;
+      tmp_bytes = 0;
+      HIPCHK(sort_pairs(st, nullptr, tmp_bytes, k_in, k_out, v_in, d.ids, m, 64));
+      DMALLOC(d_tmp, tmp_bytes);
+      HIPCHK(sort_pairs(st, d_tmp, tmp_bytes, k_in, k_out, v_in, d.ids, m, 64));
+      DBG_T("sort");
+    }
     ctx->dfree(d_tmp); d_tmp = nullptr;
     ctx->dfree(v_in);
     DMALLOC(cnt, (size_t)m * 4);
@@ -1089,24 +1140,22 @@
   uint32_t *const tab_words = reinterpret_cast<uint32_t *>(ctx->fpt);
   DBG_T("alloc+memset tab");
   if (nm) {
-    uint64_t *mv0 = nullptr, *mv1 = nullptr, *mh = nullptr, *mv = nullptr;
+    uint64_t *mv0 = nullptr, *mh = nullptr, *mv = nullptr;
     void *d_tmp = nullptr;
-    DMALLOC(mv0, std::max<uint64_t>(nk0, 1) * 8);
-    DMALLOC(mv1, std::max<uint64_t>(nk1, 1) * 8);
-    launch_iota_tag(st, mv0, nk0, 0ull);
-    launch_iota_tag(st, mv1, nk1, 1ull << 63);
     const uint64_t *h_in = nullptr, *v_in = nullptr;
     if (nk0 && nk1) {
       DMALLOC(mh, nm * 8);
       DMALLOC(mv, nm * 8);
       size_t tb = 0;
-      HIPCHK(merge_by_hash(st, nullptr, tb, uhash[0], uhash[1], mv0, mv1, mh, mv, nk0, nk1));
+      HIPCHK(merge_by_hash(st, nullptr, tb, uhash[0], uhash[1], 1ull << 63, mh, mv, nk0, nk1));
       DMALLOC(d_tmp, tb);
-      HIPCHK(merge_by_hash(st, d_tmp, tb, uhash[0], uhash[1], mv0, mv1, mh, mv, nk0, nk1));
+      HIPCHK(merge_by_hash(st, d_tmp, tb, uhash[0], uhash[1], 1ull << 63, mh, mv, nk0, nk1));
       h_in = mh; v_in = mv;
     } else {
+      DMALLOC(mv0, nm * 8);
+      launch_iota_tag(st, mv0, nm, nk0 ? 0ull : 1ull << 63);
       h_in = nk0 ? uhash[0] : uhash[1];
-      v_in = nk0 ? mv0 : mv1;
+      v_in = mv0;
     }
     DBG_T("merge");
     DictBuild db[2];
@@ -1115,12 +1164,22 @@
       db[l].ustart = ustart[l]; db[l].ucount = ucount[l]; db[l].ids = d.ids; db[l].urec = d.urec;
       db[l].deep = d.deep; db[l].ndeep = d.d_ndeep;
     }
-    uint32_t *bk_in = nullptr, *bk_out = nullptr, *d_marked = nullptr;
+    uint32_t *bk_in = nullptr, *bk_out = nullptr, *d_marked = nullptr, *d_ovf = nullptr;
     uint64_t *tp_in = nullptr, *tp_out = nullptr;
     ctx->marked_lines = 0;
     void *d_tmp2 = nullptr;
     if (!ctx->minz) {
-      launch_tab_insert(st, h_in, v_in, nm, db[0], db[1], tab_words, ctx->bshift);
+      ctx->dfree(d_tmp); d_tmp = nullptr;
+      if (nm >= 0xffffffffull) return fail(SPRING_REORDER_E_ARG, "build_dict: %llu keys exceed the 32-bit index space of the table build", (unsigned long long)nm);
+      uint32_t novf = 0;
+      DMALLOC(d_ovf, ((size_t)nm + 1) * 4);
+      HIPCHK(hipMemsetAsync(d_ovf, 0, 4, st));
+      launch_tab_insert(st, h_in, v_in, nm, db[0], db[1], tab_words, ctx->bshift, d_ovf);
+      HIPCHK(hipMemcpyAsync(&novf, d_ovf, 4, hipMemcpyDeviceToHost, st));
+      HIPCHK(hipStreamSynchronize(st));
+      DBG_T("insert pass 0");
+      launch_tab_overflow(st, h_in, v_in, nm, db[0], db[1], tab_words, ctx->bshift, d_ovf, novf);
+      if (dbg) fprintf(stderr, "[dict] %u of %llu pairs overflow their bucket\n", novf, (unsigned long long)nm);
     } else {
       DMALLOC(bk_in, nm * 4); DMALLOC(bk_out, nm * 4);
       DMALLOC(tp_in, nm * 8); DMALLOC(tp_out, nm * 8);
@@ -1148,8 +1207,8 @@
                      MID_BIN, nd[0][2], nd[1][2], BIG_BIN, nd[0][1], nd[1][1]);
     ctx->stats.table_marked_lines = ctx->marked_lines;
     DBG_T("insert");
-    ctx->dfree(mv0); ctx->dfree(mv1); ctx->dfree(mh); ctx->dfree(mv); ctx->dfree(d_tmp);
-    ctx->dfree(bk_in); ctx->dfree(bk_out); ctx->dfree(tp_in); ctx->dfree(tp_out); ctx->dfree(d_tmp2); ctx->dfree(d_marked);
+    ctx->dfree(mv0); ctx->dfree(mh); ctx->dfree(mv); ctx->dfree(d_tmp);
+    ctx->dfree(bk_in); ctx->dfree(bk_out); ctx->dfree(tp_in); ctx->dfree(tp_out); ctx->dfree(d_tmp2); ctx->dfree(d_marked); ctx->dfree(d_ovf);
   }
   for (int l = 0; l < 2; l++) { ctx->dfree(uhash[l]); ctx->dfree(ustart[l]); ctx->dfree(ucount[l]); }
   DBG_T("free temps");
diff --git a/spring_amd/reorder.py b/spring_amd/reorder.py
--- a/spring_amd/reorder.py
+++ b/spring_amd/reorder.py
@@ -42,6 +42,7 @@
     table_mode: int = 0
     phases: int = 0
     known_absent: int = 0
+    sort_prefix_bits: int = 0
 
     def to_c(self):
         o = _lib.Opts()
@@ -66,6 +67,7 @@
         o.alternatives = self.alternatives
         o.phases = self.phases
         o.known_absent = self.known_absent
+        o.sort_prefix_bits = self.sort_prefix_bits
         o.num_devices = len(self.devices)
         for i, d in enumerate(self.devices):
             o.devices[i] = d
```

New measurement: 334.3 Mreads/s (median of 6 runs). +3.0%, better.
